# NVlabs/nvbio

Hardware: NVIDIA H100
Metric: Mreads/s (150bp) seed+extend (higher is better)
Workload: dtype int32

## Files before the change

include/nvbio_b200_debug.h:

```cpp
#ifndef NVBIO_B200_DEBUG_H
#define NVBIO_B200_DEBUG_H
#include <stdint.h>
#ifdef __cplusplus
extern "C" {
#endif

void nvb_debug_force_gotoh_path(int path);
int nvb_debug_gotoh_last_route(int* packed, uint32_t* n_int32);
void nvb_debug_full_minb(int minb);
void nvb_debug_full_warp(int mode);
void nvb_debug_full_traceback_warp(int on);
void nvb_debug_pair_format(int on);
void nvb_debug_pair_rows2(int on);
void nvb_debug_traceback_fast(int on);
void nvb_debug_pair_extra_smem(int bytes);

void nvb_debug_pipeline_path(int path);

void nvb_debug_seed_split(int on);
int nvb_debug_seed_todo(uint32_t* n);

void nvb_debug_perfect_shortcut(int on);
int nvb_debug_dp_jobs(uint32_t* n);

int nvb_debug_mapq_eval(const int32_t* d_best, const uint8_t* d_has_second, const int32_t* d_second, const uint32_t* d_len,
                        const int32_t* d_match_bonus, const int32_t* d_min_score, uint32_t n, uint8_t* d_mapq, void* stream);

void nvb_debug_bgzf_grid(uint32_t ctas);

#ifdef __cplusplus
}
#endif
#endif
```

nvbio_b200/_lib.py:

```python
import ctypes as C
import os

_HERE = os.path.dirname(os.path.abspath(__file__))
LIB_PATH = os.environ.get("NVBIO_B200_LIB") or os.path.join(_HERE, "libnvbio_b200.so")

EXPORTS = [
    "nvb_version", "nvb_error_string",
    "nvb_fm_rank", "nvb_fm_rank4", "nvb_fm_match", "nvb_fm_match_approx", "nvb_fm_locate", "nvb_fm_filter_rank", "nvb_fm_filter_locate",
    "nvb_banded_gotoh_score", "nvb_banded_gotoh_score_indirect", "nvb_banded_gotoh_traceback", "nvb_gotoh_score", "nvb_gotoh_score_indirect", "nvb_banded_gotoh_score_window", "nvb_banded_gotoh_score_best2", "nvb_gotoh_traceback", "nvb_seed_extend_paired",
    "nvb_fm_build_occ", "nvb_fm_build_bwt", "nvb_fm_build_ktab", "nvb_fm_build_ktab_located", "nvb_fm_build_ktab_context", "nvb_fm_build_ktab_wide", "nvb_fm_build_rows", "nvb_seed_extend", "nvb_seed_extend_traceback", "nvb_seed_extend_mapq", "nvb_seed_extend_reseed", "nvb_seed_extend_all", "nvb_seed_extend_paired_mapq", "nvb_seed_extend_paired_traceback", "nvb_seed_extend_paired_reseed",
    "nvb_seed_extend_stage_ms",
    "nvb_dict_rank", "nvb_dict_rank4", "nvb_dict_build_occ",
    "nvb_map_seeds", "nvb_fm_locate_init", "nvb_fm_locate_lookup", "nvb_fm_locate_sorted",
    "nvb_pipeline_create", "nvb_pipeline_submit", "nvb_pipeline_wait", "nvb_pipeline_traffic", "nvb_pipeline_destroy",
    "nvb_finish_alignments", "nvb_bam_records", "nvb_bam_records_all", "nvb_bgzf_compress", "nvb_bam_sort", "nvb_bam_index", "nvb_sam_format",
]
DEBUG_EXPORTS = [
    "nvb_debug_gotoh_last_route", "nvb_debug_force_gotoh_path", "nvb_debug_full_minb", "nvb_debug_full_warp", "nvb_debug_full_traceback_warp",
    "nvb_debug_pair_format", "nvb_debug_pair_rows2", "nvb_debug_traceback_fast", "nvb_debug_pair_extra_smem",
    "nvb_debug_pipeline_path", "nvb_debug_seed_split", "nvb_debug_seed_todo", "nvb_debug_perfect_shortcut", "nvb_debug_dp_jobs", "nvb_debug_mapq_eval",
    "nvb_debug_bgzf_grid",
]


class NvbError(RuntimeError):
    pass


class FmIndexStruct(C.Structure):
    _fields_ = [("d_bwt_occ", C.c_void_p), ("d_ssa", C.c_void_p), ("length", C.c_uint32),
                ("primary", C.c_uint32), ("L2", C.c_uint32 * 5), ("sa_interval", C.c_uint32),
                ("d_ktab", C.c_void_p), ("ktab_k", C.c_uint32), ("ktab_located", C.c_uint32), ("d_rows", C.c_void_p)]


class StringSetStruct(C.Structure):
    _fields_ = [("d_words", C.c_void_p), ("bits", C.c_uint32), ("big_endian", C.c_uint32),
                ("d_offsets", C.c_void_p), ("d_lengths", C.c_void_p), ("stride", C.c_uint32),
                ("length", C.c_uint32)]


class GotohSchemeStruct(C.Structure):
    _fields_ = [("match", C.c_int32), ("mismatch", C.c_int32), ("pattern_gap_open", C.c_int32),
                ("pattern_gap_ext", C.c_int32), ("text_gap_open", C.c_int32), ("text_gap_ext", C.c_int32),
                ("d_qual_table", C.c_void_p), ("qual_table_min", C.c_int32), ("qual_table_max", C.c_int32)]


class SeedExtendParamsStruct(C.Structure):
    _fields_ = [("seed_len", C.c_uint32), ("seed_interval", C.c_uint32), ("band_len", C.c_uint32),
                ("type", C.c_uint32), ("both_strands", C.c_uint32), ("max_seed_hits", C.c_uint32),
                ("dedup_jobs", C.c_uint32), ("scheme", GotohSchemeStruct), ("d_read_quals", C.c_void_p)]


class BestAlignmentOutStruct(C.Structure):
    _fields_ = [("d_ops", C.c_void_p), ("max_ops", C.c_uint32), ("d_n_ops", C.c_void_p), ("d_begin", C.c_void_p),
                ("d_strand", C.c_void_p)]


class FinishOutStruct(C.Structure):
    _fields_ = [("d_cigar", C.c_void_p), ("max_cigar", C.c_uint32), ("d_n_cigar", C.c_void_p), ("d_md", C.c_void_p), ("max_md", C.c_uint32),
                ("d_md_len", C.c_void_p), ("d_edits", C.c_void_p)]


class BamInStruct(C.Structure):
    _fields_ = [("reads", StringSetStruct), ("d_read_quals", C.c_void_p), ("d_n_ops", C.c_void_p), ("d_begin", C.c_void_p),
                ("d_strand", C.c_void_p), ("finish", FinishOutStruct), ("d_score", C.c_void_p), ("d_mapq", C.c_void_p),
                ("d_second_score", C.c_void_p), ("d_pair_flags", C.c_void_p), ("d_contig_begin", C.c_void_p), ("n_contigs", C.c_uint32),
                ("d_names", C.c_void_p), ("d_name_offsets", C.c_void_p)]


class BamAllInStruct(C.Structure):
    _fields_ = [("base", BamInStruct), ("d_first", C.c_void_p), ("capacity", C.c_uint32)]


class BamOutStruct(C.Structure):
    _fields_ = [("d_records", C.c_void_p), ("capacity", C.c_uint64), ("d_offsets", C.c_void_p), ("d_counts", C.c_void_p)]


class BgzfOutStruct(C.Structure):
    _fields_ = [("d_out", C.c_void_p), ("capacity", C.c_uint64), ("d_block_offsets", C.c_void_p)]


class BamSortOutStruct(C.Structure):
    _fields_ = [("d_records", C.c_void_p), ("capacity", C.c_uint64), ("d_offsets", C.c_void_p), ("d_order", C.c_void_p)]


class BaiOutStruct(C.Structure):
    _fields_ = [("d_bai", C.c_void_p), ("capacity", C.c_uint64), ("d_size", C.c_void_p), ("d_status", C.c_void_p)]


class SamOutStruct(C.Structure):
    _fields_ = [("d_text", C.c_void_p), ("capacity", C.c_uint64), ("d_offsets", C.c_void_p), ("d_rejected", C.c_void_p)]


class MapqParamsStruct(C.Structure):
    _fields_ = [("d_min_score", C.c_void_p), ("max_read_len", C.c_uint32), ("match_bonus", C.c_int32)]


class MapqOutStruct(C.Structure):
    _fields_ = [("d_second_score", C.c_void_p), ("d_second_pos", C.c_void_p), ("d_second_strand", C.c_void_p), ("d_mapq", C.c_void_p)]


class ReseedParamsStruct(C.Structure):
    _fields_ = [("max_reseed", C.c_uint32), ("rep_seeds", C.c_uint32), ("d_min_score", C.c_void_p), ("max_read_len", C.c_uint32)]


class ReseedOutStruct(C.Structure):
    _fields_ = [("d_rounds", C.c_void_p), ("d_active", C.c_void_p)]


class AllParamsStruct(C.Structure):
    _fields_ = [("max_per_read", C.c_uint32), ("capacity", C.c_uint32)]


class AllOutStruct(C.Structure):
    _fields_ = [("d_first", C.c_void_p), ("d_read", C.c_void_p), ("d_score", C.c_void_p), ("d_pos", C.c_void_p),
                ("alignment", BestAlignmentOutStruct), ("d_count", C.c_void_p)]


class PairParamsStruct(C.Structure):
    _fields_ = [("min_frag", C.c_uint32), ("max_frag", C.c_uint32), ("min_mate_score", C.c_int32), ("rescue_capacity", C.c_uint32)]


class PairOutStruct(C.Structure):
    _fields_ = [("d_pair_score", C.c_void_p), ("d_pair_flags", C.c_void_p), ("d_mate_score", C.c_void_p), ("d_mate_pos", C.c_void_p),
                ("d_mate_strand", C.c_void_p), ("d_n_rescue", C.c_void_p)]


class PairMapqOutStruct(C.Structure):
    _fields_ = [("d_second_pair_score", C.c_void_p), ("d_second_mate_pos", C.c_void_p), ("d_second_mate_strand", C.c_void_p),
                ("d_mate_second_score", C.c_void_p), ("d_mate_mapq", C.c_void_p)]


class PipelineResultStruct(C.Structure):
    _fields_ = [("best_score", C.c_void_p), ("best_pos", C.c_void_p), ("n_hits", C.c_void_p), ("pair_score", C.c_void_p),
                ("pair_flags", C.c_void_p), ("mate_score", C.c_void_p), ("mate_pos", C.c_void_p), ("mate_strand", C.c_void_p),
                ("n_rescue", C.c_void_p), ("device_ms", C.c_float)]


_lib = None


def lib():
    global _lib
    if _lib is None:
        if not os.path.exists(LIB_PATH):
            raise NvbError("nvbio_b200: %s is missing -- run `python -m nvbio_b200.build` "
                           "(there is no CPU fallback)" % LIB_PATH)
        _lib = C.CDLL(LIB_PATH)
        _lib.nvb_error_string.restype = C.c_char_p
        _lib.nvb_pipeline_destroy.restype = None
        _lib.nvb_pipeline_traffic.restype = None
        for name in EXPORTS + DEBUG_EXPORTS:
            getattr(_lib, name)
    return _lib


def check(err, what=""):
    if err != 0:
        msg = lib().nvb_error_string(C.c_int(err)).decode()
        raise NvbError("%s failed: %s (%d)" % (what or "nvbio_b200 call", msg, err))
```

nvbio_b200/csrc/pipeline.cu:

```cuda
#include "fm_core.cuh"
#include "gotoh_core.cuh"
#include "pipeline_core.cuh"
#include "gotoh_full_core.cuh"
#include <cub/agent/single_pass_scan_operators.cuh>
#include <cub/block/block_scan.cuh>
#include <cub/device/device_scan.cuh>
#include <cub/device/device_select.cuh>
#include <cub/device/device_segmented_sort.cuh>
#include <mutex>

namespace nvb {

struct PipeGeom {
    uint32_t n_reads;
    uint32_t n_strings;
    uint32_t strands;
    uint32_t stride;
    uint32_t bits;
    uint32_t seeds_per_string;
    uint32_t seed_len, seed_interval;
    uint32_t band;
    uint32_t max_seed_hits;
    uint32_t genome_len;
    uint32_t seed_offset;
};

template <int BITS>
__global__ void __launch_bounds__(256)
pipe_make_strings_kernel(const StrSet reads, const PipeGeom g, uint32_t* __restrict__ out_words, uint32_t* __restrict__ out_len)
{
    constexpr uint32_t SPW = 32 / BITS;
    const uint32_t words_per_string = g.stride / SPW;
    const uint64_t t = (uint64_t)blockIdx.x * 256 + threadIdx.x;
    if (t >= (uint64_t)g.n_strings * words_per_string) return;
    const uint32_t s = (uint32_t)(t / words_per_string), w = (uint32_t)(t % words_per_string);
    const uint32_t read = s / g.strands, strand = s % g.strands;
    const uint32_t off = str_off(reads, read), len = str_len(reads, read);
    if (w == 0) out_len[s] = len;
    uint32_t word = 0;
    for (uint32_t k = 0; k < SPW; ++k) {
        const uint32_t p = w * SPW + k;
        uint32_t c = 0;
        if (p < len) {
            if (strand == 0) c = sym_at_rt(reads.words, reads.bits, reads.big_endian, off + p);
            else { c = sym_at_rt(reads.words, reads.bits, reads.big_endian, off + (len - 1u - p)); c = (c < 4u) ? 3u - c : c; }
        }
        word |= c << (32u - BITS - BITS * k);
    }
    out_words[t] = word;
}

__global__ void __launch_bounds__(256)
pipe_make_quals_kernel(const StrSet reads, const PipeGeom g, const uint8_t* __restrict__ quals, uint8_t* __restrict__ out)
{
    const uint64_t t = (uint64_t)blockIdx.x * 256 + threadIdx.x;
    if (t >= (uint64_t)g.n_strings * g.stride) return;
    const uint32_t s = (uint32_t)(t / g.stride), p = (uint32_t)(t % g.stride);
    const uint32_t read = s / g.strands, strand = s % g.strands;
    const uint32_t off = str_off(reads, read), len = str_len(reads, read);
    out[t] = (p < len) ? quals[off + (strand == 0 ? p : len - 1u - p)] : (uint8_t)0;
}

__device__ __forceinline__ uint32_t load16_2bit_be(const uint32_t* __restrict__ words, uint32_t p , uint32_t cnt )
{
    const uint32_t w = p >> 4, sh = 2u * (p & 15u);
    const uint32_t a = words[w];
    if (sh == 0) return a;
    const uint32_t b = ((p & 15u) + cnt > 16u) ? words[w + 1] : 0u;
    return (a << sh) | (b >> (32u - sh));
}
__device__ __forceinline__ uint32_t revcomp16_2bit(uint32_t x)
{
    uint32_t y = __brev(~x);
    return ((y >> 1) & 0x55555555u) | ((y & 0x55555555u) << 1);
}
__global__ void __launch_bounds__(256)
pipe_make_strings_2bit_be_kernel(const StrSet reads, const PipeGeom g, uint32_t* __restrict__ out_words, uint32_t* __restrict__ out_len)
{
    const uint32_t words_per_string = g.stride / 16u;
    const uint64_t t = (uint64_t)blockIdx.x * 256 + threadIdx.x, total = (uint64_t)g.n_strings * words_per_string;
    if (t >= total) return;
    uint32_t s, w;
    if (total <= 0xFFFFFFFFull) { s = (uint32_t)t / words_per_string; w = (uint32_t)t - s * words_per_string; }
    else                        { s = (uint32_t)(t / words_per_string); w = (uint32_t)(t % words_per_string); }
    const uint32_t read = s / g.strands, strand = s % g.strands;
    const uint32_t off = str_off(reads, read), len = str_len(reads, read);
    if (w == 0) out_len[s] = len;
    const uint32_t first = w * 16u;
    uint32_t word = 0;
    if (first < len) {
        const uint32_t cnt = (len - first) < 16u ? (len - first) : 16u;
        if (strand == 0) {
            word = load16_2bit_be(reads.words, off + first, cnt);
        } else {
            const uint32_t lo = len - first - cnt;
            uint32_t x = load16_2bit_be(reads.words, off + lo, cnt);
            x = revcomp16_2bit(x);
            word = x << (2u * (16u - cnt));
        }
        if (cnt < 16u) word &= ~(0xFFFFFFFFu >> (2u * cnt));
    }
    out_words[t] = word;
}

__device__ __forceinline__ uint32_t seed_range_hits(uint2 range, uint32_t max_seed_hits)
{
    const uint32_t sz = (range.y == 0xFFFFFFFFu) ? 1u : ((range.x <= range.y) ? (range.y - range.x + 1u) : 0u);
    return sz < max_seed_hits ? sz : max_seed_hits;
}

__device__ __forceinline__ uint2 hit_window(uint32_t pos, uint32_t seed_begin, uint32_t len, const PipeGeom& g)
{
    const uint32_t diag = pos > seed_begin ? pos - seed_begin : 0u;
    const uint32_t gb = diag > g.band / 2u ? diag - g.band / 2u : 0u;
    const uint64_t ge64 = (uint64_t)gb + len + g.band;
    return make_uint2(gb, ge64 < g.genome_len ? (uint32_t)ge64 : g.genome_len);
}

constexpr uint32_t SEED_BLOCK = 128;
constexpr uint32_t SEED_TODO_LISTS = 64;
constexpr uint32_t SEED_TODO_PITCH = 32;
constexpr uint32_t SEED_ITER = 8;
template <int BITS, bool DEFER>
__global__ void __launch_bounds__(SEED_BLOCK, 2048 / SEED_BLOCK)
pipe_seed_match_kernel(const FmIndex f, const PipeGeom g, const uint32_t* __restrict__ words, const uint32_t* __restrict__ slen,
                       const uint32_t* __restrict__ genome, uint2* __restrict__ ranges, uint32_t* __restrict__ sizes,
                       uint32_t* __restrict__ todo, uint32_t* __restrict__ todo_count)
{
    constexpr uint32_t ITER = DEFER ? SEED_ITER : 1u;
#pragma unroll 1
    for (uint32_t it = 0; it < ITER; ++it) {
        const uint32_t q = (blockIdx.x * ITER + it) * SEED_BLOCK + threadIdx.x;
        const bool live = q < g.n_strings * g.seeds_per_string;
        if (!DEFER && !live) return;
        uint32_t x = 1, y = 0;
        bool deferred = false;
        if (live) {
            const uint32_t s = q / g.seeds_per_string, k = q % g.seeds_per_string;
            const uint32_t len = slen[s];
            const uint32_t pos = g.seed_offset + k * g.seed_interval;
            if (pos + g.seed_len <= len) {
                if (genome) {
                    const uint32_t st = fm_match_locate_one<BITS, true, DEFER ? FM_DEFER : FM_WHOLE>(f, genome, words, s * g.stride + pos, g.seed_len, x, y);
                    if (st == FM_EMPTY) { x = 1; y = 0; }
                    deferred = DEFER && st == FM_DEFERRED;
                } else
                    fm_match_one<BITS, true>(f, words, s * g.stride + pos, g.seed_len, 0u, x, y);
            }
            ranges[q] = make_uint2(x, y);
            if (sizes && !deferred) sizes[q] = seed_range_hits(make_uint2(x, y), g.max_seed_hits);
        }
        if (DEFER) {
            const uint32_t m = __ballot_sync(0xFFFFFFFFu, deferred);
            if (m) {
                const uint32_t lane = threadIdx.x & 31u, list = blockIdx.x % SEED_TODO_LISTS;
                const uint32_t cap = ((gridDim.x + SEED_TODO_LISTS - 1u) / SEED_TODO_LISTS) * SEED_BLOCK * SEED_ITER;
                uint32_t base = 0;
                if (lane == 0) base = atomicAdd(todo_count + list * SEED_TODO_PITCH, (uint32_t)__popc(m));
                base = __shfl_sync(0xFFFFFFFFu, base, 0);
                if (deferred) todo[(size_t)list * cap + base + __popc(m & ((1u << lane) - 1u))] = q;
            }
        }
    }
}
template <int BITS>
__global__ void __launch_bounds__(SEED_BLOCK, 2048 / SEED_BLOCK)
pipe_seed_match_wide_kernel(const FmIndex f, const PipeGeom g, const uint32_t* __restrict__ words,
                            const uint32_t* __restrict__ genome, uint2* __restrict__ ranges, uint32_t* __restrict__ sizes,
                            const uint32_t* __restrict__ todo, const uint32_t* __restrict__ todo_count, const uint32_t seed_grid)
{
    const uint32_t list = blockIdx.x % SEED_TODO_LISTS, per_list = gridDim.x / SEED_TODO_LISTS;
    const uint32_t cap = ((seed_grid + SEED_TODO_LISTS - 1u) / SEED_TODO_LISTS) * SEED_BLOCK * SEED_ITER;
    const uint32_t n = todo_count[list * SEED_TODO_PITCH];
    for (uint32_t t = (blockIdx.x / SEED_TODO_LISTS) * SEED_BLOCK + threadIdx.x; t < n; t += per_list * SEED_BLOCK) {
        const uint32_t q = todo[(size_t)list * cap + t];
        const uint32_t s = q / g.seeds_per_string, k = q % g.seeds_per_string;
        const uint2 r = ranges[q];
        uint32_t x = r.x, y = r.y;
        if (fm_match_locate_one<BITS, true, FM_RESUME>(f, genome, words, s * g.stride + g.seed_offset + k * g.seed_interval, g.seed_len, x, y) == FM_EMPTY) { x = 1; y = 0; }
        ranges[q] = make_uint2(x, y);
        if (sizes) sizes[q] = seed_range_hits(make_uint2(x, y), g.max_seed_hits);
    }
}

__device__ __forceinline__ uint32_t upper_bound_u32(const uint32_t* __restrict__ a, uint32_t n, uint32_t v)
{
    uint32_t lo = 0, hi = n;
    while (lo < hi) { const uint32_t mid = (lo + hi) >> 1; if (a[mid] <= v) lo = mid + 1; else hi = mid; }
    return lo;
}

__global__ void pipe_count_kernel(const uint32_t* __restrict__ excl, const uint32_t* __restrict__ sizes, uint32_t n_queries, uint32_t capacity,
                                  uint32_t* __restrict__ counts)
{
    if (threadIdx.x == 0 && blockIdx.x == 0) {
        const uint32_t total = n_queries ? excl[n_queries - 1] + sizes[n_queries - 1] : 0u;
        counts[1] = total;
        counts[0] = total < capacity ? total : capacity;
    }
}

__global__ void __launch_bounds__(256)
pipe_expand_hits_kernel(const FmIndex f, const PipeGeom g, const uint2* __restrict__ ranges, const uint32_t* __restrict__ sizes,
                        const uint32_t* __restrict__ excl, const uint32_t* __restrict__ slen, const uint32_t* __restrict__ counts,
                        uint32_t* __restrict__ hit_string, uint32_t* __restrict__ p_off, uint32_t* __restrict__ p_len,
                        uint32_t* __restrict__ t_off, uint32_t* __restrict__ t_len)
{
    const uint32_t q = blockIdx.x * 256 + threadIdx.x;
    if (q >= g.n_strings * g.seeds_per_string) return;
    const uint32_t sz = sizes[q];
    if (sz == 0) return;
    const uint32_t base = excl[q], kept = counts[0];
    const uint32_t x = ranges[q].x;
    const uint32_t s = q / g.seeds_per_string, k = q % g.seeds_per_string;
    const uint32_t seed_begin = g.seed_offset + k * g.seed_interval;
    const uint32_t len = slen[s];
    for (uint32_t j = 0; j < sz; ++j) {
        const uint32_t h = base + j;
        if (h >= kept) break;
        const uint2 w = hit_window(fm_locate_one(f, x + j), seed_begin, len, g);
        hit_string[h] = s;
        p_off[h] = s * g.stride; p_len[h] = len;
        t_off[h] = w.x;          t_len[h] = w.y - w.x;
    }
}

struct Jobs { uint32_t *p_off, *p_len, *t_off, *t_len; };

constexpr uint32_t RJ_BLOCK = 128;
constexpr uint32_t RJ_STAGE = 640;
constexpr int      RJ_LOCAL = 6;
constexpr uint32_t RJ_BATCH = 4;
constexpr uint32_t RJ_CLAIMED = 0xFFFFFFFFu, RJ_CLAIMED_EMPTY = 0xFFFFFFFEu;
using RjTileState = cub::ScanTileState<uint32_t>;
using RjPrefixOp  = cub::TilePrefixCallbackOp<uint32_t, ::cuda::std::plus<uint32_t>, RjTileState>;

template <uint32_t RB>
__device__ __forceinline__ uint32_t range_batch(const uint2* __restrict__ rr, const uint32_t q0, const uint32_t n, const bool vec,
                                                const uint32_t max_seed_hits, uint32_t& hits)
{
    uint2 v[RB];
    if (vec) {
#pragma unroll
        for (uint32_t j = 0; j < RB; j += 2u) {
            const uint4 w = q0 + j < n ? *reinterpret_cast<const uint4*>(rr + q0 + j) : make_uint4(1u, 0u, 1u, 0u);
            v[j] = make_uint2(w.x, w.y); v[j + 1] = make_uint2(w.z, w.w);
        }
    } else {
#pragma unroll
        for (uint32_t j = 0; j < RB; ++j) v[j] = q0 + j < n ? rr[q0 + j] : make_uint2(1u, 0u);
    }
    uint32_t m = 0;
#pragma unroll
    for (uint32_t j = 0; j < RB; ++j) {
        const uint32_t sz = seed_range_hits(v[j], max_seed_hits);
        hits += sz;
        m |= (sz != 0u ? 1u : 0u) << j;
    }
    return m;
}

__global__ void __launch_bounds__(256)
pipe_resolve_init_kernel(RjTileState tiles, const uint32_t n_tiles, uint32_t* __restrict__ counts, uint32_t* __restrict__ dp_count)
{
    tiles.InitializeStatus((int)n_tiles);
    if (blockIdx.x == 0 && threadIdx.x == 0) { counts[2] = 0u; counts[3] = 0u; *dp_count = 0u; }
}

__global__ void __launch_bounds__(RJ_BLOCK, 8)
pipe_resolve_reads_kernel(const FmIndex f, const PipeGeom g, const uint2* __restrict__ ranges, const uint32_t* __restrict__ slen,
                          const uint32_t hit_capacity, RjTileState tiles, const uint32_t n_tiles, uint32_t* __restrict__ counts,
                          const int shortcut, const int32_t match, const int32_t mismatch, const int32_t max_gap_open,
                          const uint32_t* __restrict__ str_words, const uint32_t* __restrict__ genome,
                          uint32_t* __restrict__ j_string, uint32_t* __restrict__ j_first, const Jobs jobs,
                          int32_t* __restrict__ job_score, uint2* __restrict__ job_sink,
                          const Jobs dp, uint32_t* __restrict__ dp_job, uint32_t* __restrict__ dp_count,
                          unsigned long long* __restrict__ best_key, int32_t* best_score, uint32_t* best_pos, uint8_t* __restrict__ best_strand)
{
    using BlockScan = cub::BlockScan<uint32_t, RJ_BLOCK>;
    __shared__ struct { typename RjPrefixOp::TempStorage prefix; typename BlockScan::TempStorage scan; } s_tmp;
    __shared__ uint32_t st_string[RJ_STAGE], st_first[RJ_STAGE], st_toff[RJ_STAGE], st_tlen[RJ_STAGE], st_slot[RJ_STAGE];
    __shared__ unsigned long long s_key[RJ_BLOCK];
    __shared__ int32_t s_score[RJ_BLOCK];
    __shared__ uint32_t s_pos[RJ_BLOCK];
    __shared__ uint8_t s_strand[RJ_BLOCK];
    __shared__ uint32_t s_tile, s_cnt, s_base, s_dp_cnt, s_dp_base;
    if (threadIdx.x == 0) { s_tile = atomicAdd(counts + 3, 1u); s_cnt = 0u; s_dp_cnt = 0u; }
    s_key[threadIdx.x] = 0ull;
    __syncthreads();
    const uint32_t tile = s_tile, r0 = tile * RJ_BLOCK, r = r0 + threadIdx.x;
    const uint32_t per_read = g.strands * g.seeds_per_string;
    const bool live = r < g.n_reads;
    const uint2* rr = ranges + (size_t)r * per_read;

    const bool vec = ((per_read | (uint32_t)((size_t)ranges >> 3)) & 1u) == 0u;
    uint32_t hits = 0, run = 0, nonempty = 0;
    if (live)
        for (uint32_t q0 = 0; q0 < per_read; q0 += 16u) {
            const uint32_t m = range_batch<16>(rr, q0, per_read, vec, g.max_seed_hits, hits);
            if (q0 < 32u) nonempty |= m << q0;
        }
    if (tile == 0) {
        uint32_t aggregate;
        BlockScan(s_tmp.scan).ExclusiveSum(hits, run, aggregate);
        if (threadIdx.x == 0) tiles.SetInclusive(0, aggregate);
    } else {
        RjPrefixOp prefix(tiles, s_tmp.prefix, ::cuda::std::plus<uint32_t>{}, (int)tile);
        BlockScan(s_tmp.scan).ExclusiveSum(hits, run, prefix);
    }
    if (tile == n_tiles - 1u && threadIdx.x == RJ_BLOCK - 1u) {
        const uint32_t total = run + hits;
        counts[1] = total;
        counts[0] = total < hit_capacity ? total : hit_capacity;
    }

    if (live) {
        uint32_t lk_s[RJ_LOCAL], lk_b[RJ_LOCAL], lk_e[RJ_LOCAL];
        int n_local = 0;
        const uint32_t len0 = slen[r * g.strands], len1 = g.strands > 1u ? slen[r * g.strands + 1u] : 0u;
        for (uint32_t q0 = 0; q0 < per_read; q0 += 32u) {
            uint32_t m = q0 ? 0u : nonempty, unused = 0;
            if (q0)
                for (uint32_t b = 0; b < 32u; b += 8u) m |= range_batch<8>(rr, q0 + b, per_read, vec, g.max_seed_hits, unused) << b;
            while (m) {
                uint32_t bq[RJ_BATCH], nb = 0;
                uint2 brq[RJ_BATCH];
#pragma unroll
                for (uint32_t e = 0; e < RJ_BATCH; ++e) { bq[e] = m ? q0 + (uint32_t)__ffs(m) - 1u : 0u; nb += m ? 1u : 0u; m &= m - 1u; }
#pragma unroll
                for (uint32_t e = 0; e < RJ_BATCH; ++e) brq[e] = e < nb ? rr[bq[e]] : make_uint2(1u, 0u);
                for (uint32_t e = 0; e < nb; ++e) {
                    const uint32_t q = bq[0];
                    const uint2 rq = brq[0];
#pragma unroll
                    for (uint32_t c = 0; c + 1u < RJ_BATCH; ++c) { bq[c] = bq[c + 1]; brq[c] = brq[c + 1]; }
                    const uint32_t strand = q < g.seeds_per_string ? 0u : 1u, k = q - strand * g.seeds_per_string;
                    const uint32_t s = r * g.strands + strand, len = strand ? len1 : len0;
                    const bool located = rq.y == 0xFFFFFFFFu;
                    const uint32_t sz = seed_range_hits(rq, g.max_seed_hits);
                    const uint32_t base = run, x = rq.x, seed_begin = g.seed_offset + k * g.seed_interval;
                    run += sz;
                    for (uint32_t j = 0; j < sz; ++j) {
                        const uint32_t h = base + j;
                        if (h >= hit_capacity) break;
                        const uint2 w = hit_window(located ? x : fm_locate_one(f, x + j), seed_begin, len, g);
                        bool seen = false;
#pragma unroll
                        for (int e = 0; e < RJ_LOCAL; ++e) seen |= (e < n_local) && lk_s[e] == s && lk_b[e] == w.x && lk_e[e] == w.y;
                        if (seen) continue;
#pragma unroll
                        for (int e = 0; e < RJ_LOCAL; ++e) if (e == n_local) { lk_s[e] = s; lk_b[e] = w.x; lk_e[e] = w.y; }
                        if (n_local < RJ_LOCAL) ++n_local;
                        const uint32_t slot = atomicAdd(&s_cnt, 1u);
                        if (slot < RJ_STAGE) { st_string[slot] = s; st_first[slot] = h; st_toff[slot] = w.x; st_tlen[slot] = w.y - w.x; }
                        else {
                            const uint32_t o = atomicAdd(counts + 2, 1u), d = atomicAdd(dp_count, 1u);
                            j_string[o] = s; j_first[o] = h;
                            jobs.p_off[o] = s * g.stride; jobs.p_len[o] = len; jobs.t_off[o] = w.x; jobs.t_len[o] = w.y - w.x;
                            dp.p_off[d] = s * g.stride; dp.p_len[d] = len; dp.t_off[d] = w.x; dp.t_len[d] = w.y - w.x; dp_job[d] = o;
                        }
                    }
                }
            }
        }
    }
    __syncthreads();

    const uint32_t n = s_cnt < RJ_STAGE ? s_cnt : RJ_STAGE;
    if (threadIdx.x == 0) s_base = n ? atomicAdd(counts + 2, n) : 0u;
    __syncthreads();
    for (uint32_t i = threadIdx.x; i < n; i += RJ_BLOCK) {
        const uint32_t o = s_base + i, s = st_string[i], first = st_first[i], len = slen[s], to = st_toff[i], N = st_tlen[i];
        j_string[o] = s; j_first[o] = first; jobs.p_off[o] = s * g.stride; jobs.p_len[o] = len; jobs.t_off[o] = to; jobs.t_len[o] = N;
        int32_t score = 0; uint32_t sx = 0, sy = 0;
        if (shortcut && gapless_job_shortcut(str_words, genome, s * g.stride, len, to, N, g.band, match, mismatch, max_gap_open, score, sx, sy,
                                             shortcut != 2)) {
            const uint2 sk = make_uint2(sx, sy);
            job_score[o] = score; job_sink[o] = sk;
            if (job_aligned(sk)) {
                st_slot[i] = RJ_CLAIMED; st_toff[i] = to + sx; st_tlen[i] = (uint32_t)score;
                atomicMax(&s_key[s / g.strands - r0], make_best_key(score, first));
            } else st_slot[i] = RJ_CLAIMED_EMPTY;
        } else st_slot[i] = atomicAdd(&s_dp_cnt, 1u);
    }
    __syncthreads();
    if (threadIdx.x == 0) s_dp_base = s_dp_cnt ? atomicAdd(dp_count, s_dp_cnt) : 0u;
    __syncthreads();
    for (uint32_t i = threadIdx.x; i < n; i += RJ_BLOCK) {
        const uint32_t slot = st_slot[i], s = st_string[i];
        if (slot == RJ_CLAIMED) {
            const uint32_t rl = s / g.strands - r0;
            const int32_t score = (int32_t)st_tlen[i];
            if (s_key[rl] == make_best_key(score, st_first[i])) { s_score[rl] = score; s_pos[rl] = st_toff[i]; s_strand[rl] = (uint8_t)(s % g.strands); }
        } else if (slot != RJ_CLAIMED_EMPTY) {
            const uint32_t d = s_dp_base + slot;
            dp.p_off[d] = s * g.stride; dp.p_len[d] = slen[s]; dp.t_off[d] = st_toff[i]; dp.t_len[d] = st_tlen[i]; dp_job[d] = s_base + i;
        }
    }
    __syncthreads();
    if (live) {
        const unsigned long long key = s_key[threadIdx.x];
        best_key[r] = key;
        best_score[r] = key ? s_score[threadIdx.x] : INT_MIN;
        best_pos[r] = key ? s_pos[threadIdx.x] : 0xFFFFFFFFu;
        best_strand[r] = key ? s_strand[threadIdx.x] : (uint8_t)0;
    }
}

__global__ void __launch_bounds__(256)
pipe_scatter_dp_kernel(const PipeGeom g, const uint32_t* __restrict__ dp_count, const uint32_t* __restrict__ dp_job,
                       const int32_t* __restrict__ dp_score, const uint2* __restrict__ dp_sink,
                       const uint32_t* __restrict__ j_string, const uint32_t* __restrict__ j_first,
                       int32_t* __restrict__ job_score, uint2* __restrict__ job_sink, unsigned long long* __restrict__ best_key)
{
    const uint32_t n = *dp_count;
    for (uint32_t a = blockIdx.x * 256 + threadIdx.x; a < n; a += gridDim.x * 256) {
        const uint32_t j = dp_job[a];
        const int32_t sc = dp_score[a];
        const uint2 sk = dp_sink[a];
        job_score[j] = sc; job_sink[j] = sk;
        if (job_aligned(sk)) atomicMax(best_key + j_string[j] / g.strands, make_best_key(sc, j_first[j]));
    }
}

__global__ void __launch_bounds__(256)
pipe_finalize_dp_kernel(const PipeGeom g, const uint32_t* __restrict__ dp_count, const uint32_t* __restrict__ dp_job,
                        const int32_t* __restrict__ dp_score, const uint2* __restrict__ dp_sink, const uint32_t* __restrict__ dp_t_off,
                        const uint32_t* __restrict__ j_string, const uint32_t* __restrict__ j_first,
                        const unsigned long long* __restrict__ best_key,
                        int32_t* __restrict__ best_score, uint32_t* __restrict__ best_pos, uint8_t* __restrict__ best_strand)
{
    const uint32_t n = *dp_count;
    for (uint32_t a = blockIdx.x * 256 + threadIdx.x; a < n; a += gridDim.x * 256) {
        const uint32_t j = dp_job[a], s = j_string[j], read = s / g.strands;
        const int32_t sc = dp_score[a];
        if (best_key[read] != make_best_key(sc, j_first[j])) continue;
        best_score[read] = sc; best_pos[read] = dp_t_off[a] + dp_sink[a].x; best_strand[read] = (uint8_t)(s % g.strands);
    }
}

__global__ void __launch_bounds__(256)
pipe_find_leaders_kernel(const uint32_t* __restrict__ counts, const uint32_t* __restrict__ hit_string,
                         const uint32_t* __restrict__ t_off, const uint32_t* __restrict__ t_len,
                         uint32_t* __restrict__ leader, uint32_t* __restrict__ flag)
{
    constexpr uint32_t BACK = 64u;
    __shared__ uint32_t ss[256 + BACK], so[256 + BACK], sl[256 + BACK];
    const uint32_t n = counts[0];
    const uint32_t h0 = blockIdx.x * 256;
    if (h0 >= n) return;
    for (uint32_t i = threadIdx.x; i < 256 + BACK; i += 256) {
        const int64_t g = (int64_t)h0 - BACK + i;
        const bool in = g >= 0 && g < (int64_t)n;
        ss[i] = in ? hit_string[g] : 0xFFFFFFFFu; so[i] = in ? t_off[g] : 0u; sl[i] = in ? t_len[g] : 0u;
    }
    __syncthreads();
    const uint32_t h = h0 + threadIdx.x;
    if (h >= n) return;
    const uint32_t me = threadIdx.x + BACK;
    const uint32_t s = ss[me], o = so[me], l = sl[me];
    uint32_t lead = h;
    for (uint32_t back = 1; back <= BACK && back <= h; ++back) {
        if (ss[me - back] != s) break;
        if (so[me - back] == o && sl[me - back] == l) lead = h - back;
    }
    leader[h] = lead;
    flag[h] = (lead == h) ? 1u : 0u;
}

__global__ void pipe_job_count_kernel(const uint32_t* __restrict__ job_idx, const uint32_t* __restrict__ flag, uint32_t* __restrict__ counts)
{
    if (threadIdx.x == 0 && blockIdx.x == 0) {
        const uint32_t n = counts[0];
        counts[2] = n ? job_idx[n - 1] + flag[n - 1] : 0u;
    }
}

__global__ void __launch_bounds__(256)
pipe_compact_jobs_kernel(const uint32_t* __restrict__ counts, const uint32_t* __restrict__ flag, const uint32_t* __restrict__ job_idx,
                         const uint32_t* __restrict__ p_off, const uint32_t* __restrict__ p_len,
                         const uint32_t* __restrict__ t_off, const uint32_t* __restrict__ t_len,
                         uint32_t* __restrict__ jp_off, uint32_t* __restrict__ jp_len, uint32_t* __restrict__ jt_off, uint32_t* __restrict__ jt_len)
{
    const uint32_t h = blockIdx.x * 256 + threadIdx.x;
    if (h >= counts[0] || !flag[h]) return;
    const uint32_t j = job_idx[h];
    jp_off[j] = p_off[h]; jp_len[j] = p_len[h]; jt_off[j] = t_off[h]; jt_len[j] = t_len[h];
}

__global__ void __launch_bounds__(256)
pipe_scatter_scores_kernel(const PipeGeom g, const uint32_t* __restrict__ counts, const uint32_t* __restrict__ leader, const uint32_t* __restrict__ job_idx,
                           const int32_t* __restrict__ job_score, const uint2* __restrict__ job_sink, const uint32_t* __restrict__ hit_string,
                           int32_t* __restrict__ score, uint2* __restrict__ sink, unsigned long long* __restrict__ best_key)
{
    const uint32_t h = blockIdx.x * 256 + threadIdx.x;
    if (h >= counts[0]) return;
    uint32_t l = leader[h];
    for (uint32_t nx = leader[l]; nx != l; nx = leader[l]) l = nx;
    const uint32_t j = job_idx[l];
    const int32_t sc = job_score[j];
    const uint2 sk = job_sink[j];
    score[h] = sc;
    sink[h]  = sk;
    if (job_aligned(sk)) atomicMax(best_key + hit_string[h] / g.strands, make_best_key(sc, h));
}

__global__ void __launch_bounds__(256)
pipe_reduce_kernel(const PipeGeom g, const uint32_t* __restrict__ counts, const uint32_t* __restrict__ hit_string,
                   const int32_t* __restrict__ score, const uint2* __restrict__ sink, unsigned long long* __restrict__ best_key)
{
    const uint32_t h = blockIdx.x * 256 + threadIdx.x;
    if (h >= counts[0] || !job_aligned(sink[h])) return;
    atomicMax(best_key + hit_string[h] / g.strands, make_best_key(score[h], h));
}

__global__ void __launch_bounds__(256)
pipe_finalize_kernel(const PipeGeom g, const unsigned long long* __restrict__ best_key, const uint32_t* __restrict__ t_off,
                     const uint2* __restrict__ sink, const uint32_t* __restrict__ hit_string,
                     int32_t* __restrict__ best_score, uint32_t* __restrict__ best_pos, uint8_t* __restrict__ best_strand)
{
    const uint32_t r = blockIdx.x * 256 + threadIdx.x;
    if (r >= g.n_reads) return;
    const unsigned long long key = best_key[r];
    if (key == 0ull) { best_score[r] = INT_MIN; best_pos[r] = 0xFFFFFFFFu; if (best_strand) best_strand[r] = 0; return; }
    const uint32_t h = best_key_index(key);
    best_score[r] = best_key_score(key);
    best_pos[r] = t_off[h] + sink[h].x;
    if (best_strand) best_strand[r] = (uint8_t)(hit_string[h] % g.strands);
}

__global__ void __launch_bounds__(256)
pipe_best_jobs_kernel(const PipeGeom g, const unsigned long long* __restrict__ best_key, const uint32_t* __restrict__ hit_string,
                      const uint32_t* __restrict__ p_off, const uint32_t* __restrict__ p_len,
                      const uint32_t* __restrict__ t_off, const uint32_t* __restrict__ t_len,
                      uint32_t* __restrict__ bp_off, uint32_t* __restrict__ bp_len, uint32_t* __restrict__ bt_off, uint32_t* __restrict__ bt_len,
                      uint8_t* __restrict__ strand)
{
    const uint32_t r = blockIdx.x * 256 + threadIdx.x;
    if (r >= g.n_reads) return;
    const unsigned long long key = best_key[r];
    if (key == 0ull) { bp_off[r] = 0; bp_len[r] = 0; bt_off[r] = 0; bt_len[r] = 0; if (strand) strand[r] = 0; return; }
    const uint32_t h = best_key_index(key);
    bp_off[r] = p_off[h]; bp_len[r] = p_len[h]; bt_off[r] = t_off[h]; bt_len[r] = t_len[h];
    if (strand) strand[r] = (uint8_t)(hit_string[h] % g.strands);
}

struct Scored {
    const uint32_t* count; const uint32_t* string; const uint32_t* tie_index; Jobs jobs; const int32_t* score; const uint2* sink;
    __device__ __forceinline__ uint32_t tie(uint32_t j) const { return tie_index ? tie_index[j] : j; }
    __device__ __forceinline__ uint32_t end(uint32_t j) const { return jobs.t_off[j] + sink[j].x; }
};

__global__ void __launch_bounds__(256)
pipe_empty_jobs_kernel(const uint32_t n_reads, uint32_t* __restrict__ bp_off, uint32_t* __restrict__ bp_len, uint32_t* __restrict__ bt_off,
                       uint32_t* __restrict__ bt_len, uint8_t* __restrict__ strand)
{
    const uint32_t r = blockIdx.x * 256 + threadIdx.x;
    if (r >= n_reads) return;
    bp_off[r] = 0; bp_len[r] = 0; bt_off[r] = 0; bt_len[r] = 0;
    if (strand) strand[r] = 0;
}

__global__ void __launch_bounds__(256)
pipe_winner_kernel(const PipeGeom g, const Scored c, const unsigned long long* __restrict__ key, const Jobs out,
                   uint32_t* __restrict__ end, uint8_t* __restrict__ strand)
{
    const uint32_t n = *c.count;
    for (uint32_t j = blockIdx.x * 256 + threadIdx.x; j < n; j += gridDim.x * 256) {
        const uint32_t s = c.string[j], r = s / g.strands;
        if (key[r] != make_best_key(c.score[j], c.tie(j))) continue;
        if (out.p_off) { out.p_off[r] = c.jobs.p_off[j]; out.p_len[r] = c.jobs.p_len[j]; out.t_off[r] = c.jobs.t_off[j]; out.t_len[r] = c.jobs.t_len[j]; }
        if (end) end[r] = c.end(j);
        if (strand) strand[r] = (uint8_t)(s % g.strands);
    }
}

__global__ void __launch_bounds__(256)
traceback_begin_kernel(const uint32_t* __restrict__ d_n, const uint32_t n, const unsigned long long* __restrict__ best_key,
                       const uint32_t* __restrict__ t_off, const uint2* __restrict__ source, uint32_t* __restrict__ n_ops, uint2* __restrict__ begin)
{
    const uint32_t i = blockIdx.x * 256 + threadIdx.x;
    if (i >= (d_n ? *d_n : n)) return;
    if (best_key && best_key[i] == 0ull) { n_ops[i] = 0; begin[i] = make_uint2(0xFFFFFFFFu, 0xFFFFFFFFu); return; }
    const uint2 sc = source[i];
    begin[i] = make_uint2(t_off[i] + sc.x, sc.y);
}

__global__ void __launch_bounds__(256)
pipe_export_hits_kernel(const PipeGeom g, const uint32_t* __restrict__ counts, const uint32_t* __restrict__ hit_string,
                        const uint32_t* __restrict__ t_off, const uint32_t* __restrict__ t_len,
                        uint32_t* __restrict__ out_read, uint2* __restrict__ out_window)
{
    const uint32_t h = blockIdx.x * 256 + threadIdx.x;
    if (h >= counts[0]) return;
    if (out_read)   out_read[h] = hit_string[h];
    if (out_window) out_window[h] = make_uint2(t_off[h], t_off[h] + t_len[h]);
}


__global__ void __launch_bounds__(256)
reseed_fold_kernel(const PipeGeom g, const Scored c, const uint32_t* __restrict__ map, const uint32_t base, const uint32_t t0,
                   uint32_t* __restrict__ u_string, uint32_t* __restrict__ u_tie, const Jobs u, int32_t* __restrict__ u_score,
                   uint2* __restrict__ u_sink, unsigned long long* __restrict__ key)
{
    const uint32_t n = *c.count;
    for (uint32_t j = blockIdx.x * 256 + threadIdx.x; j < n; j += gridDim.x * 256) {
        const uint32_t s = c.string[j], read = map ? map[s / g.strands] : s / g.strands, os = read * g.strands + s % g.strands;
        const uint32_t o = base + j, tie = t0 + c.tie(j);
        const int32_t sc = c.score[j];
        const uint2 sk = c.sink[j];
        u_string[o] = os; u_tie[o] = tie;
        u.p_off[o] = os * g.stride; u.p_len[o] = c.jobs.p_len[j]; u.t_off[o] = c.jobs.t_off[j]; u.t_len[o] = c.jobs.t_len[j];
        u_score[o] = sc; u_sink[o] = sk;
        if (job_aligned(sk)) atomicMax(key + read, make_best_key(sc, tie));
    }
}

__global__ void __launch_bounds__(256)
reseed_flag_kernel(const PipeGeom g, const uint2* __restrict__ ranges, const uint32_t* __restrict__ map, const uint32_t* __restrict__ str_len,
                   const unsigned long long* __restrict__ key, const int32_t* __restrict__ min_score, const uint32_t rep_seeds,
                   uint8_t* __restrict__ flag)
{
    const uint32_t i = blockIdx.x * 256 + threadIdx.x;
    if (i >= g.n_reads) return;
    const uint32_t per_read = g.strands * g.seeds_per_string;
    const uint2* rr = ranges + (size_t)i * per_read;
    uint32_t range_sum = 0u, range_count = 0u;
    for (uint32_t q = 0; q < per_read; ++q) {
        const uint2 v = rr[q];
        if (v.y != 0xFFFFFFFFu && v.x > v.y) continue;
        range_sum += v.y == 0xFFFFFFFFu ? 1u : v.y - v.x + 1u;
        ++range_count;
    }
    bool aligned = true;
    if (min_score) {
        const unsigned long long k = key[map ? map[i] : i];
        aligned = k != 0ull && best_key_score(k) >= min_score[str_len[i * g.strands]];
    }
    flag[i] = reseed_read(range_sum, range_count, rep_seeds, aligned) ? 1u : 0u;
}

__global__ void __launch_bounds__(256)
reseed_gather_kernel(const PipeGeom g, const uint32_t* __restrict__ map, const uint32_t* __restrict__ words0, const uint32_t* __restrict__ len0,
                     const uint8_t* __restrict__ quals0, uint32_t* __restrict__ words, uint32_t* __restrict__ len, uint8_t* __restrict__ quals,
                     uint8_t* __restrict__ rounds, const uint32_t round)
{
    const uint32_t spw = 32u / g.bits, wps = g.stride / spw;
    const uint64_t t = (uint64_t)blockIdx.x * 256 + threadIdx.x;
    if (t >= (uint64_t)g.n_strings * wps) return;
    const uint32_t s = (uint32_t)(t / wps), w = (uint32_t)(t % wps), read = map[s / g.strands], os = read * g.strands + s % g.strands;
    words[t] = words0[(size_t)os * wps + w];
    if (quals)
        for (uint32_t b = 0; b < spw; ++b) quals[(size_t)s * g.stride + w * spw + b] = quals0[(size_t)os * g.stride + w * spw + b];
    if (w == 0) {
        len[s] = len0[os];
        if (rounds && s % g.strands == 0u) rounds[read] = (uint8_t)(round + 1u);
    }
}

__global__ void __launch_bounds__(256)
reseed_export_hits_kernel(const PipeGeom g, const uint32_t* __restrict__ counts, const uint32_t* __restrict__ map,
                          const uint32_t* __restrict__ hit_string, const uint32_t* __restrict__ t_off, const uint32_t* __restrict__ t_len,
                          uint32_t* __restrict__ out_read, uint2* __restrict__ out_window)
{
    const uint32_t h = blockIdx.x * 256 + threadIdx.x;
    if (h >= counts[0]) return;
    const uint32_t s = hit_string[h];
    if (out_read)   out_read[h] = (map ? map[s / g.strands] : s / g.strands) * g.strands + s % g.strands;
    if (out_window) out_window[h] = make_uint2(t_off[h], t_off[h] + t_len[h]);
}

__global__ void reseed_counts_kernel(const uint32_t* __restrict__ counts, const bool dedup, const bool per_read, uint32_t* __restrict__ totals,
                                     uint32_t* __restrict__ active, const uint32_t round, const uint32_t n_round)
{
    if (threadIdx.x != 0 || blockIdx.x != 0) return;
    const uint32_t jobs = dedup ? (counts[0] ? counts[2] : 0u) : counts[0];
    totals[0] += counts[0]; totals[1] += counts[1]; totals[2] += jobs; totals[3] += per_read ? jobs : counts[0];
    if (active) active[round] = n_round;
}

__global__ void __launch_bounds__(256)
reseed_best_kernel(const uint32_t n_reads, const unsigned long long* __restrict__ key, int32_t* __restrict__ best_score,
                   uint32_t* __restrict__ best_pos, uint8_t* __restrict__ best_strand)
{
    const uint32_t r = blockIdx.x * 256 + threadIdx.x;
    if (r >= n_reads) return;
    const unsigned long long k = key[r];
    best_score[r] = k ? best_key_score(k) : INT_MIN;
    best_pos[r] = 0xFFFFFFFFu; best_strand[r] = 0;
}

__global__ void __launch_bounds__(256) reseed_iota_kernel(const uint32_t n, uint32_t* __restrict__ map)
{
    const uint32_t i = blockIdx.x * 256 + threadIdx.x;
    if (i < n) map[i] = i;
}


__device__ __forceinline__ bool second_candidate(int32_t score, uint32_t end, uint32_t strand, uint32_t len, uint32_t best_end,
                                                 uint32_t best_strand, const int32_t* __restrict__ min_score)
{
    return score >= min_score[len] && distinct_alignment(end, strand, best_end, best_strand, len);
}

__global__ void __launch_bounds__(256)
pipe_second_reduce_kernel(const PipeGeom g, const Scored c, const uint32_t* __restrict__ str_len, const uint32_t* __restrict__ best_pos,
                          const uint8_t* __restrict__ best_strand, const int32_t* __restrict__ min_score,
                          unsigned long long* __restrict__ second_key)
{
    const uint32_t n = *c.count;
    for (uint32_t j = blockIdx.x * 256 + threadIdx.x; j < n; j += gridDim.x * 256) {
        const uint32_t s = c.string[j], read = s / g.strands;
        const int32_t sc = c.score[j];
        if (job_aligned(c.sink[j]) && second_candidate(sc, c.end(j), s % g.strands, str_len[s], best_pos[read], best_strand[read], min_score))
            atomicMax(second_key + read, make_best_key(sc, c.tie(j)));
    }
}

__global__ void __launch_bounds__(256)
pipe_mapq_kernel(const PipeGeom g, const nvb_mapq_params mp, const uint32_t* __restrict__ str_len, const int32_t* __restrict__ best_score,
                 const unsigned long long* __restrict__ second_key, int32_t* __restrict__ second_score, uint32_t* __restrict__ second_pos,
                 uint8_t* __restrict__ second_strand, uint8_t* __restrict__ mapq)
{
    const uint32_t r = blockIdx.x * 256 + threadIdx.x;
    if (r >= g.n_reads) return;
    const unsigned long long key = second_key[r];
    const bool has = key != 0ull;
    const int32_t s2 = has ? best_key_score(key) : INT_MIN;
    second_score[r] = s2;
    if (!has) {
        if (second_pos) second_pos[r] = 0xFFFFFFFFu;
        if (second_strand) second_strand[r] = 0;
    }
    const uint32_t len = str_len[r * g.strands];
    mapq[r] = (uint8_t)bowtie_mapq2(best_score[r], has, s2, (int32_t)len * mp.match_bonus, mp.d_min_score[len], mp.match_bonus == 0);
}

__global__ void __launch_bounds__(256)
debug_mapq_eval_kernel(const int32_t* __restrict__ best, const uint8_t* __restrict__ has_second, const int32_t* __restrict__ second,
                       const uint32_t* __restrict__ len, const int32_t* __restrict__ match_bonus, const int32_t* __restrict__ min_score,
                       uint32_t n, uint8_t* __restrict__ mapq)
{
    const uint32_t i = blockIdx.x * 256 + threadIdx.x;
    if (i >= n) return;
    mapq[i] = (uint8_t)bowtie_mapq2(best[i], has_second[i] != 0, second[i], (int32_t)len[i] * match_bonus[i], min_score[i], match_bonus[i] == 0);
}

__global__ void __launch_bounds__(256)
cand_scatter_kernel(const PipeGeom g, const Scored c, const uint32_t* __restrict__ str_len, const int32_t* __restrict__ min_score,
                    const uint32_t* __restrict__ seg, uint32_t* __restrict__ cursor, unsigned long long* __restrict__ key,
                    uint32_t* __restrict__ val, const bool by_best)
{
    const uint32_t n = *c.count;
    for (uint32_t j = blockIdx.x * 256 + threadIdx.x; j < n; j += gridDim.x * 256) {
        const uint32_t s = c.string[j], read = s / g.strands;
        if (!reportable(c.score[j], c.sink[j], min_score[str_len[s]])) continue;
        const uint32_t slot = atomicAdd(cursor + read, 1u);
        if (!seg) continue;
        key[seg[read] + slot] = by_best ? ~make_best_key(c.score[j], c.tie(j)) : ((unsigned long long)(s % g.strands) << 32) | c.end(j);
        val[seg[read] + slot] = j;
    }
}


__global__ void __launch_bounds__(256)
all_select_kernel(const PipeGeom g, const Scored c, const uint32_t* __restrict__ str_len, const uint32_t* __restrict__ seg,
                  unsigned long long* __restrict__ es, uint32_t* __restrict__ idx, const uint32_t k, uint32_t* __restrict__ cnt)
{
    const uint32_t r = blockIdx.x * 256 + threadIdx.x;
    if (r >= g.n_reads) return;
    const uint32_t b = seg[r], n = seg[r + 1] - b;
    for (uint32_t i = 0; i < n; ++i) {
        const uint32_t j = idx[b + i];
        es[b + i] = end_strand(c.end(j), c.string[j] % g.strands);
    }
    cnt[r] = select_distinct(es + b, idx + b, n, str_len[r * g.strands], k);
}

__global__ void __launch_bounds__(256)
all_count_kernel(const uint32_t n_reads, const uint32_t* __restrict__ first, const uint32_t capacity, const uint32_t n_slices,
                 uint32_t* __restrict__ count, uint32_t* __restrict__ slice_n)
{
    const uint32_t stored = first[upper_bound_u32(first, n_reads + 1u, capacity) - 1u];
    const uint32_t t = blockIdx.x * 256 + threadIdx.x;
    if (t == 0) { count[0] = stored; count[1] = first[n_reads]; }
    if (t >= n_slices) return;
    const uint64_t b = (uint64_t)t * n_reads;
    slice_n[t] = stored > b ? (uint32_t)(stored - b < n_reads ? stored - b : n_reads) : 0u;
}

__global__ void __launch_bounds__(256)
all_emit_kernel(const PipeGeom g, const Scored c, const uint32_t* __restrict__ first, const uint32_t* __restrict__ seg,
                const uint32_t* __restrict__ idx, const uint32_t capacity, uint32_t* __restrict__ out_read, int32_t* __restrict__ out_score,
                uint32_t* __restrict__ out_pos, uint8_t* __restrict__ out_strand, const Jobs jobs)
{
    const uint32_t r = blockIdx.x * 256 + threadIdx.x;
    if (r >= g.n_reads) return;
    const uint32_t o = first[r], e = first[r + 1];
    if (e > capacity) return;
    const uint32_t* sel = idx + seg[r];
    for (uint32_t a = o; a < e; ++a) {
        const uint32_t j = sel[a - o], s = c.string[j];
        out_read[a] = r; out_score[a] = c.score[j]; out_pos[a] = c.end(j); out_strand[a] = (uint8_t)(s % g.strands);
        jobs.p_off[a] = c.jobs.p_off[j]; jobs.p_len[a] = c.jobs.p_len[j]; jobs.t_off[a] = c.jobs.t_off[j]; jobs.t_len[a] = c.jobs.t_len[j];
    }
}

struct MateBest { bool has; int32_t score; uint32_t strand, beg, end, len; };

__device__ __forceinline__ MateBest mate_best(const PipeGeom& g, uint32_t r, const int32_t* best_score,
                                              const uint32_t* best_pos, const uint8_t* __restrict__ best_strand,
                                              const uint32_t* __restrict__ str_len)
{
    MateBest m; m.has = false; m.score = INT_MIN; m.strand = 0; m.beg = m.end = 0xFFFFFFFFu; m.len = 0;
    const uint32_t end = best_pos[r];
    if (end == 0xFFFFFFFFu) return m;
    m.has = true;
    m.score = best_score[r];
    m.strand = best_strand[r];
    m.len = str_len[r * g.strands];
    m.end = end;
    m.beg = aln_begin(m.end, m.len);
    return m;
}

__global__ void __launch_bounds__(256)
pair_classify_kernel(const PipeGeom g, const uint32_t n_pairs, const nvb_pair_params pp,
                     const int32_t* best_score, const uint32_t* best_pos, const uint8_t* __restrict__ best_strand,
                     const uint32_t* __restrict__ str_len,
                     uint32_t* __restrict__ want, uint32_t* __restrict__ w_pstr, uint32_t* __restrict__ w_toff, uint32_t* __restrict__ w_tlen,
                     int32_t* __restrict__ pair_score, uint32_t* __restrict__ pair_flags,
                     int32_t* mate_score, uint32_t* mate_pos, uint8_t* __restrict__ mate_strand)
{
    const uint32_t p = blockIdx.x * 256 + threadIdx.x;
    if (p >= n_pairs) return;
    MateBest m[2];
    m[0] = mate_best(g, p, best_score, best_pos, best_strand, str_len);
    m[1] = mate_best(g, n_pairs + p, best_score, best_pos, best_strand, str_len);
#pragma unroll
    for (int k = 0; k < 2; ++k) {
        mate_score[k * n_pairs + p] = m[k].score; mate_pos[k * n_pairs + p] = m[k].end; mate_strand[k * n_pairs + p] = (uint8_t)m[k].strand;
    }
    bool conc = m[0].has && m[1].has && (m[0].strand != m[1].strand);
    if (conc) {
        const MateBest& f = m[0].strand == 0 ? m[0] : m[1];
        const MateBest& r = m[0].strand == 0 ? m[1] : m[0];
        conc = fr_concordant(f.beg, f.end, r.beg, r.end, pp.min_frag, pp.max_frag);
    }
    if (conc) {
        pair_score[p] = m[0].score + m[1].score; pair_flags[p] = NVB_PAIR_CONCORDANT;
        want[2 * p] = want[2 * p + 1] = 0u;
        return;
    }
    pair_score[p] = INT_MIN; pair_flags[p] = NVB_PAIR_UNPAIRED;
#pragma unroll
    for (int a = 0; a < 2; ++a) {
        uint32_t w = 0u, ps = 0u, to = 0u, tl = 0u;
        if (m[a].has && m[a].score >= pp.min_mate_score) {
            const uint32_t o_read = (uint32_t)(1 - a) * n_pairs + p;
            if (m[a].strand == 0u) { to = m[a].beg; const uint32_t e = (g.genome_len - to) < pp.max_frag ? g.genome_len : to + pp.max_frag; tl = e - to; ps = 2u * o_read + 1u; }
            else                   { to = m[a].end > pp.max_frag ? m[a].end - pp.max_frag : 0u; tl = m[a].end - to; ps = 2u * o_read; }
            w = (tl >= 1u && str_len[ps] >= 1u) ? 1u : 0u;
        }
        want[2 * p + a] = w; w_pstr[2 * p + a] = ps; w_toff[2 * p + a] = to; w_tlen[2 * p + a] = tl;
    }
}

__global__ void __launch_bounds__(256)
pair_compact_kernel(const PipeGeom g, const uint32_t n_slots, const uint32_t capacity, const uint32_t* __restrict__ want, const uint32_t* __restrict__ job_idx,
                    const uint32_t* __restrict__ w_pstr, const uint32_t* __restrict__ w_toff, const uint32_t* __restrict__ w_tlen,
                    const uint32_t* __restrict__ str_len,
                    uint32_t* __restrict__ jp_off, uint32_t* __restrict__ jp_len, uint32_t* __restrict__ jt_off, uint32_t* __restrict__ jt_len)
{
    const uint32_t i = blockIdx.x * 256 + threadIdx.x;
    if (i >= n_slots || !want[i]) return;
    const uint32_t j = job_idx[i];
    if (j >= capacity) return;
    jp_off[j] = w_pstr[i] * g.stride; jp_len[j] = str_len[w_pstr[i]]; jt_off[j] = w_toff[i]; jt_len[j] = w_tlen[i];
}

__device__ __forceinline__ bool usable_rescue(const nvb_pair_params& pp, const uint32_t* __restrict__ want, const uint32_t* __restrict__ job_idx,
                                              const uint32_t* __restrict__ w_toff, const int32_t* __restrict__ rs_score,
                                              const uint2* __restrict__ rs_sink, uint32_t i, int32_t& score, uint32_t& end)
{
    if (!want[i]) return false;
    const uint32_t j = job_idx[i];
    if (j >= pp.rescue_capacity) return false;
    score = rs_score[j];
    if (score < pp.min_mate_score) return false;
    end = w_toff[i] + rs_sink[j].x;
    return true;
}

__global__ void __launch_bounds__(256)
pair_finalize_kernel(const uint32_t n_pairs, const nvb_pair_params pp, const uint32_t* __restrict__ want, const uint32_t* __restrict__ job_idx,
                     const uint32_t* __restrict__ w_toff, const int32_t* __restrict__ rs_score, const uint2* __restrict__ rs_sink,
                     int32_t* __restrict__ pair_score, uint32_t* __restrict__ pair_flags,
                     int32_t* __restrict__ mate_score, uint32_t* __restrict__ mate_pos, uint8_t* __restrict__ mate_strand)
{
    const uint32_t p = blockIdx.x * 256 + threadIdx.x;
    if (p >= n_pairs || pair_flags[p] == NVB_PAIR_CONCORDANT) return;
    int best_a = -1; int32_t best_sum = INT_MIN, best_rs = 0; uint32_t best_pos = 0;
#pragma unroll
    for (int a = 0; a < 2; ++a) {
        int32_t rs; uint32_t end;
        if (!usable_rescue(pp, want, job_idx, w_toff, rs_score, rs_sink, 2 * p + a, rs, end)) continue;
        const int32_t sum = mate_score[a * n_pairs + p] + rs;
        if (sum > best_sum) { best_sum = sum; best_a = a; best_rs = rs; best_pos = end; }
    }
    if (best_a < 0) return;
    const int o = 1 - best_a;
    pair_score[p] = best_sum;
    pair_flags[p] = o == 0 ? NVB_PAIR_RESCUED_MATE1 : NVB_PAIR_RESCUED_MATE2;
    mate_score[o * n_pairs + p] = best_rs;
    mate_pos[o * n_pairs + p] = best_pos;
    mate_strand[o * n_pairs + p] = (uint8_t)(1u - mate_strand[best_a * n_pairs + p]);
}

__device__ __forceinline__ bool pair_rescued(uint32_t flags) { return flags == NVB_PAIR_RESCUED_MATE1 || flags == NVB_PAIR_RESCUED_MATE2; }

__global__ void __launch_bounds__(256)
pair_empty_rescued_jobs_kernel(const uint32_t n_pairs, const uint32_t* __restrict__ pair_flags, uint32_t* __restrict__ bp_len, uint32_t* __restrict__ bt_len)
{
    const uint32_t p = blockIdx.x * 256 + threadIdx.x;
    if (p >= n_pairs) return;
    const uint32_t f = pair_flags[p];
    if (!pair_rescued(f)) return;
    const uint32_t r = (f == NVB_PAIR_RESCUED_MATE1 ? 0u : n_pairs) + p;
    bp_len[r] = 0; bt_len[r] = 0;
}

__global__ void __launch_bounds__(256)
pair_rescue_items_kernel(const uint32_t n_pairs, const uint32_t* __restrict__ pair_flags, const uint32_t* __restrict__ job_idx,
                         const uint8_t* __restrict__ mate_strand, uint2* __restrict__ items, uint32_t* __restrict__ n_items, uint8_t* __restrict__ ba_strand)
{
    const uint32_t p = blockIdx.x * 256 + threadIdx.x, lane = threadIdx.x & 31u;
    const uint32_t f = p < n_pairs ? pair_flags[p] : 0u;
    const bool rescued = pair_rescued(f);
    const uint32_t m = __ballot_sync(0xFFFFFFFFu, rescued);
    if (!m) return;
    uint32_t base = 0;
    if (lane == 0) base = atomicAdd(n_items, (uint32_t)__popc(m));
    base = __shfl_sync(0xFFFFFFFFu, base, 0);
    if (!rescued) return;
    const uint32_t o = f == NVB_PAIR_RESCUED_MATE1 ? 0u : 1u, out = o * n_pairs + p;
    items[base + __popc(m & ((1u << lane) - 1u))] = make_uint2(job_idx[2u * p + (1u - o)], out);
    if (ba_strand) ba_strand[out] = mate_strand[out];
}


__global__ void __launch_bounds__(256)
pair_cand_merge_kernel(const uint32_t n_reads, const uint32_t* __restrict__ seg, const uint32_t* __restrict__ cnt,
                       const unsigned long long* __restrict__ key, const uint32_t* __restrict__ val, const Scored c,
                       uint32_t* __restrict__ m_end, int32_t* __restrict__ m_score, uint32_t* __restrict__ m_tie,
                       uint32_t* __restrict__ n_fw, uint32_t* __restrict__ n_merged)
{
    const uint32_t r = blockIdx.x * 256 + threadIdx.x;
    if (r >= n_reads) return;
    const uint32_t b = seg[r], n = cnt[r];
    uint32_t m = 0, fw = 0; unsigned long long prev = ~0ull;
    for (uint32_t k = b; k < b + n; ++k) {
        const unsigned long long kk = key[k];
        const uint32_t j = val[k], tie = c.tie(j);
        const int32_t sc = c.score[j];
        if (kk == prev) {
            const uint32_t o = b + m - 1u;
            if (sc > m_score[o] || (sc == m_score[o] && tie < m_tie[o])) { m_score[o] = sc; m_tie[o] = tie; }
            continue;
        }
        prev = kk;
        m_end[b + m] = (uint32_t)kk; m_score[b + m] = sc; m_tie[b + m] = tie;
        ++m; if ((kk >> 32) == 0ull) ++fw;
    }
    n_fw[r] = fw; n_merged[r] = m;
}

__global__ void __launch_bounds__(256)
pair_second_kernel(const uint32_t n_pairs, const nvb_pair_params pp, const nvb_mapq_params mp, const uint32_t* __restrict__ str_len,
                   const uint32_t* __restrict__ seg, const uint32_t* __restrict__ n_fw, const uint32_t* __restrict__ n_merged,
                   const uint32_t* __restrict__ m_end, const int32_t* __restrict__ m_score, const uint32_t* __restrict__ m_tie,
                   const uint32_t* __restrict__ se_pos, const uint8_t* __restrict__ se_strand, const unsigned long long* __restrict__ best_key,
                   const uint32_t* __restrict__ want, const uint32_t* __restrict__ job_idx, const uint32_t* __restrict__ w_toff,
                   const int32_t* __restrict__ rs_score, const uint2* __restrict__ rs_sink,
                   const int32_t* __restrict__ pair_score, const uint32_t* __restrict__ pair_flags,
                   const uint32_t* __restrict__ mate_pos, const uint8_t* __restrict__ mate_strand,
                   int32_t* __restrict__ second_pair_score, uint32_t* __restrict__ second_mate_pos, uint8_t* __restrict__ second_mate_strand,
                   uint8_t* __restrict__ mate_mapq)
{
    const uint32_t p = blockIdx.x * 256 + threadIdx.x;
    if (p >= n_pairs) return;
    const uint32_t r0 = p, r1 = n_pairs + p;
    const uint32_t len[2] = {str_len[2u * r0], str_len[2u * r1]};
    PairSecond ps;
    ps.init(mate_pos[r0], mate_strand[r0], len[0], mate_pos[r1], mate_strand[r1], len[1]);
    const uint32_t flags = pair_flags[p];
    if (flags != NVB_PAIR_UNPAIRED) {
        MateCands m[2];
#pragma unroll
        for (int k = 0; k < 2; ++k) {
            const uint32_t r = k ? r1 : r0, b = seg[r];
            m[k].end = m_end + b; m[k].score = m_score + b; m[k].tie = m_tie + b; m[k].n_fw = n_fw[r]; m[k].n = n_merged[r]; m[k].len = len[k];
        }
        pair_combinations(m, pp.min_frag, pp.max_frag, ps);
        for (int a = 0; a < 2; ++a) {
            const uint32_t ra = a ? r1 : r0;
            int32_t rs; uint32_t end;
            if (!usable_rescue(pp, want, job_idx, w_toff, rs_score, rs_sink, 2u * p + a, rs, end) || rs < mp.d_min_score[len[1 - a]]) continue;
            const unsigned long long key = best_key[ra];
            ps.offer_rescue(a, best_key_score(key) + rs, se_pos[ra], se_strand[ra], best_key_index(key), end);
        }
        const uint8_t q = (uint8_t)bowtie_mapq2(pair_score[p], ps.has, ps.score, (int32_t)(len[0] + len[1]) * mp.match_bonus,
                                                mp.d_min_score[len[0]] + mp.d_min_score[len[1]], mp.match_bonus == 0);
        mate_mapq[r0] = q; mate_mapq[r1] = q;
    }
    second_pair_score[p] = ps.score;
#pragma unroll
    for (int k = 0; k < 2; ++k) {
        if (second_mate_pos) second_mate_pos[k * n_pairs + p] = ps.end[k];
        if (second_mate_strand) second_mate_strand[k * n_pairs + p] = (uint8_t)ps.strand[k];
    }
}

}

using namespace nvb;

struct StageEvents { cudaEvent_t ev[8]; bool ready, valid; };
static StageEvents g_stage[NVB_MAX_DEVICES];
static std::mutex  g_stage_mutex;
static int default_stage_events(StageEvents** out)
{
    int dev = 0;
    NVB_CUDA_TRY(cudaGetDevice(&dev));
    if (dev < 0 || dev >= NVB_MAX_DEVICES) return NVB_E_UNSUPPORTED;
    std::lock_guard<std::mutex> lock(g_stage_mutex);
    StageEvents& S = g_stage[dev];
    if (!S.ready) {
        for (int i = 0; i < 8; ++i) NVB_CUDA_TRY(cudaEventCreate(&S.ev[i]));
        S.ready = true;
    }
    *out = &S;
    return NVB_OK;
}

extern "C" int nvb_seed_extend_stage_ms(float ms[7])
{
    if (!ms) return NVB_E_INVALID;
    StageEvents* SE = nullptr;
    { const int r = default_stage_events(&SE); if (r != NVB_OK) return r; }
    if (!SE->valid) return NVB_E_INVALID;
    NVB_CUDA_TRY(cudaEventSynchronize(SE->ev[7]));
    for (int i = 0; i < 7; ++i) NVB_CUDA_TRY(cudaEventElapsedTime(&ms[i], SE->ev[i], SE->ev[i + 1]));
    return NVB_OK;
}

static int g_perfect_shortcut = 1;
static const uint32_t* g_last_dp_count = nullptr;
static int g_seed_split = 1;
static const uint32_t* g_last_seed_todo = nullptr;
static int g_pipe_path = 0;

#define NVB_TRY(expr) do { const int _r = (expr); if (_r != NVB_OK) return _r; } while (0)
static int size_only(int r) { return r == NVB_E_TEMP_SIZE ? NVB_OK : r; }
static int launched() { return (int)cudaGetLastError(); }

static uint32_t resident_grid(uint32_t n) { const uint32_t grid = (n + 255) / 256, cap = sm_count() * 16u; return grid < cap ? grid : cap; }

static Jobs take_jobs(TempCarver& tc, size_t n) { return Jobs{tc.take<uint32_t>(n), tc.take<uint32_t>(n), tc.take<uint32_t>(n), tc.take<uint32_t>(n)}; }
struct JobViews { nvb_string_set pats, txts; };

struct SeedExtendReq {
    const nvb_fm_index* fmi; const uint32_t* genome; const nvb_string_set* reads; uint32_t n_reads; const nvb_seed_extend_params* P; uint32_t hit_capacity;
    int32_t* best_score; uint32_t* best_pos; uint32_t* n_hits; uint32_t* hit_read; nvb_uint2* hit_window; int32_t* hit_score; nvb_uint2* hit_sink;
    const nvb_best_alignment_out* BA; const nvb_pair_params* PP; const nvb_pair_out* PO;
    const nvb_mapq_params* MP; const nvb_mapq_out* MO; const nvb_pair_mapq_out* PMO;
    const nvb_all_params* AP; const nvb_all_out* AO;
};

struct PipeCall : SeedExtendReq {
    PipeGeom g; cudaStream_t s; FmIndex f; StrSet rd;
    uint32_t nq;
    bool dedup, per_read, eligible;
    bool seed_split;
    nvb_mapq_out se_mo;
    StageEvents* SE;
    uint32_t *str_words, *str_len; uint8_t* str_quals;
    uint2* ranges; uint32_t *sizes, *excl, *counts, *seed_todo, *seed_todo_n;
    char* rj_tiles; size_t rj_tile_bytes;
    uint32_t *j_string, *j_first;
    uint32_t *leader, *flag, *job_idx;
    Jobs jobs; int32_t* job_score; uint2* job_sink;
    Jobs dp; uint32_t *dp_job, *dp_count; int32_t* dp_score; uint2* dp_sink;
    uint32_t* hit_string; Jobs hits; int32_t* h_score; uint2* h_sink;
    unsigned long long* best_key; uint8_t* rb_strand;
    char *scan_tmp, *gotoh_tmp; size_t scan_bytes, gotoh_bytes;
    Jobs best; int32_t* b_score; uint2 *b_sink, *b_source; char* tb_tmp; size_t tb_bytes;
    uint32_t *pw_want, *pw_idx, *pw_pstr, *pw_toff, *pw_tlen, *pcounts;
    Jobs rescue; int32_t* rs_score; uint2* rs_sink; char *pscan_tmp, *full_tmp; size_t pscan_bytes, full_bytes;
    uint2* rt_items; uint32_t* rt_count; char* rt_pool; size_t rt_pool_bytes;
    unsigned long long* second_key;
    uint32_t *cs_cnt, *cs_seg, *cs_val[2]; unsigned long long* cs_key[2];
    char *cs_scan_tmp, *cs_sort_tmp; size_t cs_scan_bytes, cs_sort_bytes;
    uint32_t *pc_fw, *pc_n, *pc_end, *pc_tie, *se_pos; int32_t* pc_score;
    uint32_t *al_slice_n, n_slices; Jobs al_jobs;
    const Scored* uni;

    int stage(int i) const { return (int)cudaEventRecord(SE->ev[i], s); }

    JobViews job_views(const Jobs& j, uint32_t txt_len) const
    {
        return {{str_words ? str_words : (const uint32_t*)16,  g.bits, 1u,         j.p_off,   j.p_len,   0u,     rd.length},
                {genome,                                       2u,     1u,         j.t_off,   j.t_len,   0u,     txt_len}};
    }

    int score_jobs(const Jobs& j, const uint32_t* d_n, int32_t* score, uint2* sink) const
    {
        const JobViews v = job_views(j, rd.length + g.band);
        size_t bytes = gotoh_bytes;
        return nvb_banded_gotoh_score_indirect(g.band, P->type, &P->scheme, &v.pats, str_quals, &v.txts, d_n, hit_capacity,
                                               score, (nvb_uint2*)sink, gotoh_tmp, &bytes, s);
    }

    int carve(void* d_temp, size_t& need)
    {
        const uint32_t cap = hit_capacity, n_reads = g.n_reads;
        const JobViews sv = job_views(Jobs{}, rd.length + g.band);
        NVB_TRY(size_only(nvb_banded_gotoh_score(g.band, P->type, &P->scheme, &sv.pats, nullptr, &sv.txts, cap, nullptr, nullptr, nullptr,
                                                 &gotoh_bytes, s)));
        TempCarver tc(d_temp);
        str_words = tc.take<uint32_t>((size_t)g.n_strings * (g.stride / (32u / g.bits)) + 4);
        str_len   = tc.take<uint32_t>(g.n_strings);
        str_quals = P->d_read_quals ? tc.take<uint8_t>((size_t)g.n_strings * g.stride + 16) : nullptr;
        ranges = tc.take<uint2>(nq);
        if (!per_read) { sizes = tc.take<uint32_t>(nq); excl = tc.take<uint32_t>(nq); }
        if (seed_split) seed_todo = tc.take<uint32_t>((size_t)nq + (SEED_TODO_LISTS + 1u) * SEED_BLOCK * SEED_ITER);
        counts = tc.take<uint32_t>(4); seed_todo_n = tc.take<uint32_t>(SEED_TODO_LISTS * SEED_TODO_PITCH);
        if (per_read) {
            NVB_CUDA_TRY(RjTileState::AllocationSize((int)((n_reads + RJ_BLOCK - 1u) / RJ_BLOCK), rj_tile_bytes));
            rj_tiles = tc.take<char>(rj_tile_bytes);
        }
        if (per_read) { j_string = tc.take<uint32_t>(cap); j_first = tc.take<uint32_t>(cap); }
        else if (dedup) { leader = tc.take<uint32_t>(cap); flag = tc.take<uint32_t>(cap); job_idx = tc.take<uint32_t>(cap); }
        if (dedup) { jobs = take_jobs(tc, cap); job_score = tc.take<int32_t>(cap); job_sink = tc.take<uint2>(cap); }
        if (per_read) {
            dp = take_jobs(tc, cap); dp_job = tc.take<uint32_t>(cap); dp_score = tc.take<int32_t>(cap); dp_sink = tc.take<uint2>(cap);
            dp_count = tc.take<uint32_t>(4);
        }
        if (!per_read) { hit_string = tc.take<uint32_t>(cap); hits = take_jobs(tc, cap); }
        h_score = hit_score ? hit_score : (per_read ? nullptr : tc.take<int32_t>(cap));
        h_sink  = hit_sink ? (uint2*)hit_sink : (per_read ? nullptr : tc.take<uint2>(cap));
        best_key = tc.take<unsigned long long>(n_reads); rb_strand = tc.take<uint8_t>((size_t)n_reads + 16);
        scan_bytes = 0;
        if (!per_read) NVB_CUDA_TRY(cub::DeviceScan::ExclusiveSum(nullptr, scan_bytes, sizes, excl, (int)nq, s));
        if (dedup && !per_read && cap) {
            size_t scan2_bytes = 0;
            NVB_CUDA_TRY(cub::DeviceScan::ExclusiveSum(nullptr, scan2_bytes, flag, job_idx, (int)cap, s));
            if (scan2_bytes > scan_bytes) scan_bytes = scan2_bytes;
        }
        scan_tmp  = tc.take<char>(scan_bytes);
        gotoh_tmp = tc.take<char>(gotoh_bytes);
        if (BA || AO) {
            if (BA) best = take_jobs(tc, n_reads);
            b_score = tc.take<int32_t>(n_reads); b_sink = tc.take<uint2>(n_reads); b_source = tc.take<uint2>(n_reads);
            NVB_TRY(size_only(nvb_banded_gotoh_traceback(g.band, P->type, &P->scheme, &sv.pats, nullptr, &sv.txts, n_reads, nullptr, nullptr,
                                                         nullptr, nullptr, BA ? BA->max_ops : AO->alignment.max_ops, nullptr, nullptr, &tb_bytes, s)));
            tb_tmp = tc.take<char>(tb_bytes);
        }
        if (PP) {
            const uint32_t rcap = PP->rescue_capacity;
            pw_want = tc.take<uint32_t>(n_reads); pw_idx = tc.take<uint32_t>(n_reads); pw_pstr = tc.take<uint32_t>(n_reads);
            pw_toff = tc.take<uint32_t>(n_reads); pw_tlen = tc.take<uint32_t>(n_reads); pcounts = tc.take<uint32_t>(4);
            rescue = take_jobs(tc, rcap); rs_score = tc.take<int32_t>(rcap); rs_sink = tc.take<uint2>(rcap);
            NVB_CUDA_TRY(cub::DeviceScan::ExclusiveSum(nullptr, pscan_bytes, pw_want, pw_idx, (int)n_reads, s));
            pscan_tmp = tc.take<char>(pscan_bytes);
            const JobViews v = job_views(Jobs{}, PP->max_frag);
            NVB_TRY(size_only(nvb_gotoh_score_indirect(P->type, &P->scheme, &v.pats, nullptr, &v.txts, (const uint32_t*)16, rcap, nullptr, nullptr,
                                                       nullptr, &full_bytes, s)));
            full_tmp = tc.take<char>(full_bytes);
            if (BA) {
                NVB_TRY(full_warp_traceback(P->type, rd.length, PP->max_frag, nullptr, &rt_pool_bytes, s));
                rt_items = tc.take<uint2>((size_t)n_reads / 2u + 1u); rt_count = tc.take<uint32_t>(4); rt_pool = tc.take<char>(rt_pool_bytes);
            }
        }
        if (MO) second_key = tc.take<unsigned long long>(n_reads);
        if (PMO || AO) {
            cs_cnt = tc.take<uint32_t>((size_t)n_reads + 1); cs_seg = tc.take<uint32_t>((size_t)n_reads + 1);
            for (int k = 0; k < 2; ++k) { cs_key[k] = tc.take<unsigned long long>(cap); cs_val[k] = tc.take<uint32_t>(cap); }
            NVB_CUDA_TRY(cub::DeviceScan::ExclusiveSum(nullptr, cs_scan_bytes, cs_cnt, cs_seg, (int)n_reads + 1, s));
            cs_scan_tmp = tc.take<char>(cs_scan_bytes);
            cs_sort_bytes = 0;
            if (cap) NVB_CUDA_TRY(cub::DeviceSegmentedSort::SortPairs(nullptr, cs_sort_bytes, cs_key[0], cs_key[1], cs_val[0], cs_val[1], (int)cap,
                                                                     (int)n_reads, cs_seg, cs_seg + 1, s));
            cs_sort_tmp = tc.take<char>(cs_sort_bytes);
        }
        if (PMO) {
            if (!PMO->d_mate_second_score) se_mo.d_second_score = tc.take<int32_t>(n_reads);
            pc_fw = tc.take<uint32_t>(n_reads); pc_n = tc.take<uint32_t>(n_reads); se_pos = tc.take<uint32_t>(n_reads);
            pc_end = tc.take<uint32_t>(cap); pc_score = tc.take<int32_t>(cap); pc_tie = tc.take<uint32_t>(cap);
        }
        if (AO) {
            const uint32_t acap = AP->capacity;
            n_slices = n_reads ? (uint32_t)(((uint64_t)acap + n_reads - 1u) / n_reads) : 0u;
            al_jobs = take_jobs(tc, acap); al_slice_n = tc.take<uint32_t>((size_t)n_slices + 1);
        }
        need = tc.total();
        return NVB_OK;
    }

    int make_strings() const
    {
        const uint32_t grid = (uint32_t)(((uint64_t)g.n_strings * (g.stride / (32u / g.bits)) + 255) / 256);
        if (g.bits == 2 && rd.big_endian) pipe_make_strings_2bit_be_kernel<<<grid, 256, 0, s>>>(rd, g, str_words, str_len);
        else if (g.bits == 2)             pipe_make_strings_kernel<2><<<grid, 256, 0, s>>>(rd, g, str_words, str_len);
        else                              pipe_make_strings_kernel<4><<<grid, 256, 0, s>>>(rd, g, str_words, str_len);
        NVB_LAUNCH_CHECK();
        if (str_quals) pipe_make_quals_kernel<<<(uint32_t)(((uint64_t)g.n_strings * g.stride + 255) / 256), 256, 0, s>>>(rd, g, P->d_read_quals, str_quals);
        return launched();
    }

    int match_seeds() const
    {
        const uint32_t grid = (nq + SEED_BLOCK - 1) / SEED_BLOCK;
        const uint32_t* loc_genome = (per_read && f.sa_shift == 0u) ? genome : nullptr;
        if (seed_split) {
            NVB_CUDA_TRY(cudaMemsetAsync(seed_todo_n, 0, SEED_TODO_LISTS * SEED_TODO_PITCH * sizeof(uint32_t), s));
            const uint32_t grid1 = (grid + SEED_ITER - 1u) / SEED_ITER;
            if (g.bits == 2) pipe_seed_match_kernel<2, true><<<grid1, SEED_BLOCK, 0, s>>>(f, g, str_words, str_len, loc_genome, ranges, sizes, seed_todo, seed_todo_n);
            else             pipe_seed_match_kernel<4, true><<<grid1, SEED_BLOCK, 0, s>>>(f, g, str_words, str_len, loc_genome, ranges, sizes, seed_todo, seed_todo_n);
            NVB_LAUNCH_CHECK();
            const uint32_t wgrid = (sm_count() * 16u + SEED_TODO_LISTS - 1u) / SEED_TODO_LISTS * SEED_TODO_LISTS;
            if (g.bits == 2) pipe_seed_match_wide_kernel<2><<<wgrid, SEED_BLOCK, 0, s>>>(f, g, str_words, loc_genome, ranges, sizes, seed_todo, seed_todo_n, grid1);
            else             pipe_seed_match_wide_kernel<4><<<wgrid, SEED_BLOCK, 0, s>>>(f, g, str_words, loc_genome, ranges, sizes, seed_todo, seed_todo_n, grid1);
            g_last_seed_todo = seed_todo_n;
        } else {
            if (g.bits == 2) pipe_seed_match_kernel<2, false><<<grid, SEED_BLOCK, 0, s>>>(f, g, str_words, str_len, loc_genome, ranges, sizes, nullptr, nullptr);
            else             pipe_seed_match_kernel<4, false><<<grid, SEED_BLOCK, 0, s>>>(f, g, str_words, str_len, loc_genome, ranges, sizes, nullptr, nullptr);
        }
        return launched();
    }

    int hit_slots() const
    {
        if (per_read) return NVB_OK;
        size_t bytes = scan_bytes;
        NVB_CUDA_TRY(cub::DeviceScan::ExclusiveSum(scan_tmp, bytes, sizes, excl, (int)nq, s));
        pipe_count_kernel<<<1, 32, 0, s>>>(excl, sizes, nq, hit_capacity, counts);
        return launched();
    }

    int extend_per_read() const
    {
        const nvb_gotoh_scheme& SC = P->scheme;
        const uint32_t cap = hit_capacity, n_tiles = (g.n_reads + RJ_BLOCK - 1u) / RJ_BLOCK;
        RjTileState tiles;
        NVB_CUDA_TRY(tiles.Init((int)n_tiles, rj_tiles, rj_tile_bytes));
        pipe_resolve_init_kernel<<<(n_tiles + 255u) / 256u, 256, 0, s>>>(tiles, n_tiles, counts, dp_count);
        NVB_LAUNCH_CHECK();
        const int shortcut = eligible ? g_perfect_shortcut : 0;
        const int32_t max_gap_open = SC.pattern_gap_open > SC.text_gap_open ? SC.pattern_gap_open : SC.text_gap_open;
        pipe_resolve_reads_kernel<<<n_tiles, RJ_BLOCK, 0, s>>>(f, g, ranges, str_len, cap, tiles, n_tiles, counts, shortcut, SC.match,
                SC.mismatch, max_gap_open, str_words, genome, j_string, j_first, jobs, job_score, job_sink, dp, dp_job, dp_count,
                best_key, best_score, best_pos, rb_strand);
        NVB_LAUNCH_CHECK();
        g_last_dp_count = dp_count;
        NVB_TRY(stage(4)); NVB_TRY(stage(5));
        const uint32_t jgrid = resident_grid(cap);
        if (cap) {
            NVB_TRY(score_jobs(dp, dp_count, dp_score, dp_sink));
            pipe_scatter_dp_kernel<<<jgrid, 256, 0, s>>>(g, dp_count, dp_job, dp_score, dp_sink, j_string, j_first, job_score, job_sink, best_key);
            NVB_LAUNCH_CHECK();
        }
        NVB_TRY(stage(6));
        if (cap) {
            pipe_finalize_dp_kernel<<<jgrid, 256, 0, s>>>(g, dp_count, dp_job, dp_score, dp_sink, dp.t_off, j_string, j_first, best_key,
                                                          best_score, best_pos, rb_strand);
            NVB_LAUNCH_CHECK();
        }
        return launched();
    }

    int extend_per_hit() const
    {
        const uint32_t cap = hit_capacity, hgrid = (cap + 255) / 256;
        if (cap) {
            pipe_expand_hits_kernel<<<(nq + 255) / 256, 256, 0, s>>>(f, g, ranges, sizes, excl, str_len, counts,
                                                                     hit_string, hits.p_off, hits.p_len, hits.t_off, hits.t_len);
            NVB_LAUNCH_CHECK();
        }
        NVB_TRY(stage(4));
        if (dedup && cap) {
            pipe_find_leaders_kernel<<<hgrid, 256, 0, s>>>(counts, hit_string, hits.t_off, hits.t_len, leader, flag);
            NVB_LAUNCH_CHECK();
            size_t bytes = scan_bytes;
            NVB_CUDA_TRY(cub::DeviceScan::ExclusiveSum(scan_tmp, bytes, flag, job_idx, (int)cap, s));
            pipe_job_count_kernel<<<1, 32, 0, s>>>(job_idx, flag, counts);
            NVB_LAUNCH_CHECK();
            pipe_compact_jobs_kernel<<<hgrid, 256, 0, s>>>(counts, flag, job_idx, hits.p_off, hits.p_len, hits.t_off, hits.t_len,
                                                           jobs.p_off, jobs.p_len, jobs.t_off, jobs.t_len);
            NVB_LAUNCH_CHECK();
        }
        NVB_TRY(stage(5));
        NVB_CUDA_TRY(cudaMemsetAsync(best_key, 0, sizeof(unsigned long long) * g.n_reads, s));
        if (cap && dedup) {
            NVB_TRY(score_jobs(jobs, counts + 2, job_score, job_sink));
            pipe_scatter_scores_kernel<<<hgrid, 256, 0, s>>>(g, counts, leader, job_idx, job_score, job_sink, hit_string, h_score, h_sink, best_key);
            NVB_LAUNCH_CHECK();
        } else if (cap)
            NVB_TRY(score_jobs(hits, counts, h_score, h_sink));
        NVB_TRY(stage(6));
        if (cap && !dedup) {
            pipe_reduce_kernel<<<hgrid, 256, 0, s>>>(g, counts, hit_string, h_score, h_sink, best_key);
            NVB_LAUNCH_CHECK();
        }
        pipe_finalize_kernel<<<(g.n_reads + 255) / 256, 256, 0, s>>>(g, best_key, hits.t_off, h_sink, hit_string, best_score, best_pos, rb_strand);
        return launched();
    }

    int best_traceback() const
    {
        const uint32_t rgrid = (g.n_reads + 255) / 256;
        if (per_read || uni) {
            pipe_empty_jobs_kernel<<<rgrid, 256, 0, s>>>(g.n_reads, best.p_off, best.p_len, best.t_off, best.t_len, BA->d_strand);
            NVB_LAUNCH_CHECK();
            const uint32_t jgrid = resident_grid(hit_capacity);
            if (jgrid) {
                pipe_winner_kernel<<<jgrid, 256, 0, s>>>(g, scored(), best_key, best, nullptr, BA->d_strand);
                NVB_LAUNCH_CHECK();
            }
        } else {
            pipe_best_jobs_kernel<<<rgrid, 256, 0, s>>>(g, best_key, hit_string, hits.p_off, hits.p_len, hits.t_off, hits.t_len,
                                                        best.p_off, best.p_len, best.t_off, best.t_len, BA->d_strand);
            NVB_LAUNCH_CHECK();
        }
        if (PP) {
            const uint32_t n_pairs = g.n_reads / 2u;
            pair_empty_rescued_jobs_kernel<<<(n_pairs + 255) / 256, 256, 0, s>>>(n_pairs, PO->d_pair_flags, best.p_len, best.t_len);
            NVB_LAUNCH_CHECK();
        }
        return trace_jobs(best, nullptr, g.n_reads, *BA, 0, best_key);
    }

    int trace_jobs(const Jobs& j, const uint32_t* d_n, uint32_t n, const nvb_best_alignment_out& A, size_t off, const unsigned long long* key) const
    {
        const JobViews v = job_views(j, rd.length + g.band);
        size_t bytes = tb_bytes;
        NVB_TRY(banded_traceback(g.band, P->type, &P->scheme, &v.pats, str_quals, &v.txts, d_n, n, b_score, (nvb_uint2*)b_sink,
                                 (nvb_uint2*)b_source, A.d_ops + off * A.max_ops, A.max_ops, A.d_n_ops + off, tb_tmp, &bytes, s));
        traceback_begin_kernel<<<(n + 255) / 256, 256, 0, s>>>(d_n, n, key, j.t_off, b_source, A.d_n_ops + off, (uint2*)A.d_begin + off);
        return launched();
    }

    Scored scored() const
    {
        if (uni) return *uni;
        return per_read ? Scored{counts + 2, j_string, j_first, jobs, job_score, job_sink} : Scored{counts, hit_string, nullptr, hits, h_score, h_sink};
    }

    int second_best() const
    {
        NVB_CUDA_TRY(cudaMemsetAsync(second_key, 0, sizeof(unsigned long long) * g.n_reads, s));
        if (hit_capacity) {
            const uint32_t grid = resident_grid(hit_capacity);
            pipe_second_reduce_kernel<<<grid, 256, 0, s>>>(g, scored(), str_len, best_pos, rb_strand, MP->d_min_score, second_key);
            NVB_LAUNCH_CHECK();
            if (MO->d_second_pos || MO->d_second_strand) {
                pipe_winner_kernel<<<grid, 256, 0, s>>>(g, scored(), second_key, Jobs{}, MO->d_second_pos, MO->d_second_strand);
                NVB_LAUNCH_CHECK();
            }
        }
        pipe_mapq_kernel<<<(g.n_reads + 255) / 256, 256, 0, s>>>(g, *MP, str_len, best_score, second_key, MO->d_second_score, MO->d_second_pos,
                                                                MO->d_second_strand, MO->d_mapq);
        return launched();
    }

    int cand_segments(bool by_best) const
    {
        const uint32_t cap = hit_capacity, n_reads = g.n_reads;
        NVB_CUDA_TRY(cudaMemsetAsync(cs_cnt, 0, sizeof(uint32_t) * ((size_t)n_reads + 1), s));
        if (cap) {
            const uint32_t grid = resident_grid(cap);
            cand_scatter_kernel<<<grid, 256, 0, s>>>(g, scored(), str_len, MP->d_min_score, nullptr, cs_cnt, nullptr, nullptr, by_best);
            NVB_LAUNCH_CHECK();
            size_t bytes = cs_scan_bytes;
            NVB_CUDA_TRY(cub::DeviceScan::ExclusiveSum(cs_scan_tmp, bytes, cs_cnt, cs_seg, (int)n_reads + 1, s));
            NVB_CUDA_TRY(cudaMemsetAsync(cs_cnt, 0, sizeof(uint32_t) * n_reads, s));
            cand_scatter_kernel<<<grid, 256, 0, s>>>(g, scored(), str_len, MP->d_min_score, cs_seg, cs_cnt, cs_key[0], cs_val[0], by_best);
            NVB_LAUNCH_CHECK();
            bytes = cs_sort_bytes;
            NVB_CUDA_TRY(cub::DeviceSegmentedSort::SortPairs(cs_sort_tmp, bytes, cs_key[0], cs_key[1], cs_val[0], cs_val[1], (int)cap, (int)n_reads,
                                                             cs_seg, cs_seg + 1, s));
        } else
            NVB_CUDA_TRY(cudaMemsetAsync(cs_seg, 0, sizeof(uint32_t) * ((size_t)n_reads + 1), s));
        return NVB_OK;
    }

    int pair_candidates() const
    {
        NVB_CUDA_TRY(cudaMemcpyAsync(se_pos, best_pos, sizeof(uint32_t) * g.n_reads, cudaMemcpyDeviceToDevice, s));
        NVB_TRY(cand_segments(false));
        pair_cand_merge_kernel<<<(g.n_reads + 255) / 256, 256, 0, s>>>(g.n_reads, cs_seg, cs_cnt, cs_key[1], cs_val[1], scored(), pc_end, pc_score,
                                                                        pc_tie, pc_fw, pc_n);
        return launched();
    }

    int all_alignments() const
    {
        const uint32_t n_reads = g.n_reads, acap = AP->capacity, rgrid = (n_reads + 255) / 256;
        const nvb_all_out& O = *AO;
        NVB_TRY(cand_segments(true));
        all_select_kernel<<<rgrid, 256, 0, s>>>(g, scored(), str_len, cs_seg, cs_key[1], cs_val[1], AP->max_per_read, cs_cnt);
        NVB_LAUNCH_CHECK();
        size_t bytes = cs_scan_bytes;
        NVB_CUDA_TRY(cub::DeviceScan::ExclusiveSum(cs_scan_tmp, bytes, cs_cnt, O.d_first, (int)n_reads + 1, s));
        all_count_kernel<<<(n_slices + 256) / 256, 256, 0, s>>>(n_reads, O.d_first, acap, n_slices, O.d_count, al_slice_n);
        NVB_LAUNCH_CHECK();
        if (!acap) return launched();
        all_emit_kernel<<<rgrid, 256, 0, s>>>(g, scored(), O.d_first, cs_seg, cs_val[1], acap, O.d_read, O.d_score, O.d_pos, O.alignment.d_strand,
                                              al_jobs);
        NVB_LAUNCH_CHECK();
        for (uint32_t t = 0; t < n_slices; ++t) {
            const size_t b = (size_t)t * n_reads;
            const Jobs j{al_jobs.p_off + b, al_jobs.p_len + b, al_jobs.t_off + b, al_jobs.t_len + b};
            NVB_TRY(trace_jobs(j, al_slice_n + t, (uint32_t)(acap - b < n_reads ? acap - b : n_reads), O.alignment, b, nullptr));
        }
        return launched();
    }

    int pair_second() const
    {
        const uint32_t n_pairs = g.n_reads / 2u;
        pair_second_kernel<<<(n_pairs + 255) / 256, 256, 0, s>>>(n_pairs, *PP, *MP, str_len, cs_seg, pc_fw, pc_n, pc_end, pc_score, pc_tie,
                                                                  se_pos, rb_strand, best_key, pw_want, pw_idx, pw_toff, rs_score, rs_sink,
                                                                  PO->d_pair_score, PO->d_pair_flags, PO->d_mate_pos, PO->d_mate_strand,
                                                                  PMO->d_second_pair_score, PMO->d_second_mate_pos, PMO->d_second_mate_strand,
                                                                  PMO->d_mate_mapq);
        return launched();
    }

    int paired_rescue() const
    {
        const uint32_t n_reads = g.n_reads, n_pairs = n_reads / 2u, cap = PP->rescue_capacity;
        const uint32_t pgrid = (n_pairs + 255) / 256, sgrid = (n_reads + 255) / 256;
        pair_classify_kernel<<<pgrid, 256, 0, s>>>(g, n_pairs, *PP, best_score, best_pos, rb_strand, str_len, pw_want, pw_pstr, pw_toff, pw_tlen,
                                                    PO->d_pair_score, PO->d_pair_flags, PO->d_mate_score, PO->d_mate_pos, PO->d_mate_strand);
        NVB_LAUNCH_CHECK();
        size_t bytes = pscan_bytes;
        NVB_CUDA_TRY(cub::DeviceScan::ExclusiveSum(pscan_tmp, bytes, pw_want, pw_idx, (int)n_reads, s));
        pipe_count_kernel<<<1, 32, 0, s>>>(pw_idx, pw_want, n_reads, cap, pcounts);
        NVB_LAUNCH_CHECK();
        if (cap) {
            pair_compact_kernel<<<sgrid, 256, 0, s>>>(g, n_reads, cap, pw_want, pw_idx, pw_pstr, pw_toff, pw_tlen, str_len,
                                                      rescue.p_off, rescue.p_len, rescue.t_off, rescue.t_len);
            NVB_LAUNCH_CHECK();
            const JobViews v = job_views(rescue, PP->max_frag);
            size_t fb = full_bytes;
            NVB_TRY(nvb_gotoh_score_indirect(P->type, &P->scheme, &v.pats, str_quals, &v.txts, pcounts, cap, rs_score, (nvb_uint2*)rs_sink, full_tmp, &fb, s));
        }
        pair_finalize_kernel<<<pgrid, 256, 0, s>>>(n_pairs, *PP, pw_want, pw_idx, pw_toff, rs_score, rs_sink, PO->d_pair_score, PO->d_pair_flags,
                                                    PO->d_mate_score, PO->d_mate_pos, PO->d_mate_strand);
        NVB_LAUNCH_CHECK();
        if (PO->d_n_rescue) NVB_CUDA_TRY(cudaMemcpyAsync(PO->d_n_rescue, pcounts, 2 * sizeof(uint32_t), cudaMemcpyDeviceToDevice, s));
        return NVB_OK;
    }

    int after_extension(const uint32_t* hit_counts) const
    {
        if (BA && !PP) NVB_TRY(best_traceback());
        if (MO) NVB_TRY(second_best());
        if (AO) NVB_TRY(all_alignments());
        if (PMO) NVB_TRY(pair_candidates());
        if (PP) NVB_TRY(paired_rescue());
        if (BA && PP) { NVB_TRY(best_traceback()); NVB_TRY(rescue_traceback()); }
        if (PMO) NVB_TRY(pair_second());
        if (n_hits) NVB_CUDA_TRY(cudaMemcpyAsync(n_hits, hit_counts, 3 * sizeof(uint32_t), cudaMemcpyDeviceToDevice, s));
        NVB_TRY(stage(7));
        SE->valid = true;
        return NVB_OK;
    }

    int rescue_traceback() const
    {
        const uint32_t n_pairs = g.n_reads / 2u;
        NVB_CUDA_TRY(cudaMemsetAsync(rt_count, 0, sizeof(uint32_t), s));
        pair_rescue_items_kernel<<<(n_pairs + 255) / 256, 256, 0, s>>>(n_pairs, PO->d_pair_flags, pw_idx, PO->d_mate_strand, rt_items, rt_count,
                                                                       BA->d_strand);
        NVB_LAUNCH_CHECK();
        const JobViews v = job_views(rescue, PP->max_frag);
        FullTbArgs a;
        a.S = make_scheme(&P->scheme); a.pat = make_strset(&v.pats); a.txt = make_strset(&v.txts); a.quals = str_quals;
        a.score = rs_score; a.sink = rs_sink; a.items = rt_items; a.n_items = rt_count;
        a.o.ops = BA->d_ops; a.o.n_ops = BA->d_n_ops; a.o.source = (uint2*)BA->d_begin; a.o.max_ops = BA->max_ops; a.o.absolute = 1u;
        a.pool = rt_pool;
        size_t bytes = rt_pool_bytes;
        return full_warp_traceback(P->type, rd.length, PP->max_frag, &a, &bytes, s);
    }
};

struct ReseedCall {
    const nvb_reseed_params* RP; const nvb_reseed_out* RO;
    uint32_t *map[2], *totals; uint8_t* flag; unsigned long long* key;
    uint32_t *r_words, *r_len; uint8_t* r_quals;
    uint32_t *u_string, *u_tie; Jobs u; int32_t* u_score; uint2* u_sink;
    char* sel_tmp; size_t sel_bytes;

    int carve(const PipeCall& c, void* base, size_t& need)
    {
        const uint32_t n = c.g.n_reads, cap = c.hit_capacity;
        TempCarver tc(base);
        map[0] = tc.take<uint32_t>(n); map[1] = tc.take<uint32_t>(n); flag = tc.take<uint8_t>((size_t)n + 16);
        totals = tc.take<uint32_t>(8); key = tc.take<unsigned long long>(n);
        r_words = tc.take<uint32_t>((size_t)c.g.n_strings * (c.g.stride / (32u / c.g.bits)) + 4); r_len = tc.take<uint32_t>(c.g.n_strings);
        r_quals = c.P->d_read_quals ? tc.take<uint8_t>((size_t)c.g.n_strings * c.g.stride + 16) : nullptr;
        u_string = tc.take<uint32_t>(cap); u_tie = tc.take<uint32_t>(cap); u = take_jobs(tc, cap);
        u_score = tc.take<int32_t>(cap); u_sink = tc.take<uint2>(cap);
        sel_bytes = 0;
        NVB_CUDA_TRY(cub::DeviceSelect::Flagged(nullptr, sel_bytes, map[0], flag, map[1], totals + 4, (int)n, c.s));
        sel_tmp = tc.take<char>(sel_bytes);
        need = tc.total();
        return NVB_OK;
    }

    int run(PipeCall& c)
    {
        const cudaStream_t s = c.s;
        const PipeGeom g0 = c.g;
        const uint32_t n = g0.n_reads, cap = c.hit_capacity, n_rounds = RP->max_reseed + 1u;
        uint32_t* const words0 = c.str_words; uint32_t* const len0 = c.str_len; uint8_t* const quals0 = c.str_quals;
        int32_t* const h_score0 = c.h_score; uint2* const h_sink0 = c.h_sink;
        uint8_t* const rounds = RO ? RO->d_rounds : nullptr; uint32_t* const active = RO ? RO->d_active : nullptr;
        const uint32_t rgrid = (n + 255) / 256;
        NVB_CUDA_TRY(cudaMemsetAsync(totals, 0, 8 * sizeof(uint32_t), s));
        NVB_CUDA_TRY(cudaMemsetAsync(key, 0, sizeof(unsigned long long) * n, s));
        if (rounds) NVB_CUDA_TRY(cudaMemsetAsync(rounds, 1, n, s));
        if (active) NVB_CUDA_TRY(cudaMemsetAsync(active, 0, sizeof(uint32_t) * n_rounds, s));
        reseed_iota_kernel<<<rgrid, 256, 0, s>>>(n, map[0]);
        NVB_LAUNCH_CHECK();
        NVB_TRY(default_stage_events(&c.SE));
        NVB_TRY(c.stage(0));
        NVB_TRY(c.make_strings()); NVB_TRY(c.stage(1));
        uint32_t n_r = n, host[5] = {0u, 0u, 0u, 0u, 0u};
        int cur = 0;
        for (uint32_t r = 0; r < n_rounds && n_r; ++r) {
            const uint32_t kept = host[0], base = host[3];
            c.g.n_reads = n_r; c.g.n_strings = n_r * g0.strands; c.nq = c.g.n_strings * g0.seeds_per_string;
            c.g.seed_offset = reseed_offset(r, g0.seed_interval, RP->max_reseed);
            if (r) {
                reseed_gather_kernel<<<(uint32_t)(((uint64_t)c.g.n_strings * (g0.stride / (32u / g0.bits)) + 255) / 256), 256, 0, s>>>(
                    c.g, map[cur], words0, len0, quals0, r_words, r_len, quals0 ? r_quals : nullptr, rounds, r);
                NVB_LAUNCH_CHECK();
                c.str_words = r_words; c.str_len = r_len; c.str_quals = quals0 ? r_quals : nullptr;
            }
            c.hit_capacity = cap - kept;
            c.h_score = c.hit_score ? c.hit_score + kept : h_score0;
            c.h_sink = c.hit_sink ? (uint2*)c.hit_sink + kept : h_sink0;
            NVB_TRY(c.match_seeds()); NVB_TRY(c.stage(2));
            NVB_TRY(c.hit_slots());   NVB_TRY(c.stage(3));
            NVB_TRY(c.per_read ? c.extend_per_read() : c.extend_per_hit());
            if (c.hit_capacity) {
                if (c.hit_read || c.hit_window) {
                    reseed_export_hits_kernel<<<(c.hit_capacity + 255) / 256, 256, 0, s>>>(c.g, c.counts, map[cur], c.hit_string, c.hits.t_off,
                        c.hits.t_len, c.hit_read ? c.hit_read + kept : nullptr, c.hit_window ? (uint2*)c.hit_window + kept : nullptr);
                    NVB_LAUNCH_CHECK();
                }
                reseed_fold_kernel<<<resident_grid(c.hit_capacity), 256, 0, s>>>(c.g, c.scored(), map[cur], base, kept, u_string, u_tie, u,
                                                                                  u_score, u_sink, key);
                NVB_LAUNCH_CHECK();
            }
            reseed_counts_kernel<<<1, 32, 0, s>>>(c.counts, c.dedup, c.per_read, totals, active, r, n_r);
            NVB_LAUNCH_CHECK();
            if (r + 1u == n_rounds) break;
            reseed_flag_kernel<<<(n_r + 255) / 256, 256, 0, s>>>(c.g, c.ranges, map[cur], c.str_len, key, c.PP ? nullptr : RP->d_min_score,
                                                                 RP->rep_seeds, flag);
            NVB_LAUNCH_CHECK();
            size_t bytes = sel_bytes;
            NVB_CUDA_TRY(cub::DeviceSelect::Flagged(sel_tmp, bytes, map[cur], flag, map[cur ^ 1], totals + 4, (int)n_r, s));
            NVB_CUDA_TRY(cudaMemcpyAsync(host, totals, sizeof(host), cudaMemcpyDeviceToHost, s));
            NVB_CUDA_TRY(cudaStreamSynchronize(s));
            n_r = host[4]; cur ^= 1;
        }
        c.g = g0; c.str_words = words0; c.str_len = len0; c.str_quals = quals0; c.hit_capacity = cap;
        const Scored U{totals + 3, u_string, u_tie, u, u_score, u_sink};
        c.uni = &U; c.best_key = key;
        reseed_best_kernel<<<rgrid, 256, 0, s>>>(n, key, c.best_score, c.best_pos, c.rb_strand);
        NVB_LAUNCH_CHECK();
        if (cap) {
            pipe_winner_kernel<<<resident_grid(cap), 256, 0, s>>>(g0, U, key, Jobs{}, c.best_pos, c.rb_strand);
            NVB_LAUNCH_CHECK();
        }
        return c.after_extension(totals);
    }
};

static int seed_extend_impl(const SeedExtendReq& R, void* d_temp, size_t* temp_bytes, void* stream, ReseedCall* RS = nullptr)
{
    if (!R.reads || !temp_bytes) return NVB_E_INVALID;
    if (R.BA && (!R.BA->d_ops || !R.BA->d_n_ops || !R.BA->d_begin || R.BA->max_ops == 0)) return NVB_E_INVALID;
    if ((R.MP == nullptr) != (R.MO == nullptr && R.PMO == nullptr)) return NVB_E_INVALID;
    if (R.MP && (!R.MP->d_min_score || R.MP->max_read_len < R.reads->length)) return NVB_E_INVALID;
    if (R.MO && (!R.MO->d_second_score || !R.MO->d_mapq)) return NVB_E_INVALID;
    if (R.PMO && (!R.PMO->d_second_pair_score || !R.PMO->d_mate_mapq)) return NVB_E_INVALID;
    if (R.PP && R.BA && R.reads->length > FULL_TB_MAX_M) return NVB_E_UNSUPPORTED;
    if (R.AO && R.reads->length > FULL_TB_MAX_M) return NVB_E_UNSUPPORTED;
    const nvb_seed_extend_params* P = R.P;
    if (R.PP) {
        if (!R.PO->d_pair_score || !R.PO->d_pair_flags || !R.PO->d_mate_score || !R.PO->d_mate_pos || !R.PO->d_mate_strand) return NVB_E_INVALID;
        if (!P || !P->both_strands || (R.n_reads & 1u) || R.PP->max_frag == 0 || R.PP->min_frag > R.PP->max_frag) return NVB_E_INVALID;
    }
    if (!valid_fmindex(R.fmi) || !R.fmi->d_ssa || !R.genome || !valid_strset(R.reads) || !P) return NVB_E_INVALID;
    if (R.reads->bits == 8) return NVB_E_UNSUPPORTED;
    if (P->seed_len == 0 || P->seed_interval == 0 || P->max_seed_hits == 0) return NVB_E_INVALID;
    if (R.n_reads && (!R.best_score || !R.best_pos)) return NVB_E_INVALID;
    const uint32_t max_len = R.reads->length;
    if (max_len < P->seed_len) return NVB_E_INVALID;

    PipeCall c{R};
    PipeGeom& g = c.g;
    g.n_reads = R.n_reads; g.strands = P->both_strands ? 2u : 1u; g.n_strings = R.n_reads * g.strands;
    g.bits = R.reads->bits;
    const uint32_t spw = 32u / g.bits;
    g.stride = (max_len + spw - 1u) / spw * spw;
    g.seeds_per_string = (max_len - P->seed_len) / P->seed_interval + 1u;
    g.seed_len = P->seed_len; g.seed_interval = P->seed_interval; g.band = P->band_len;
    g.max_seed_hits = P->max_seed_hits; g.genome_len = R.fmi->length;
    if ((uint64_t)g.n_strings * g.stride > 0xFFFFFFFFull) return NVB_E_UNSUPPORTED;
    const uint64_t nq64 = (uint64_t)g.n_strings * g.seeds_per_string;
    if (nq64 > 0x7FFFFFFFull) return NVB_E_UNSUPPORTED;
    if (nq64 * (uint64_t)P->max_seed_hits > 0xFFFFFFFFull) return NVB_E_UNSUPPORTED;

    const cudaStream_t s = c.s = as_stream(stream);
    c.f = make_fmindex(R.fmi); c.rd = make_strset(R.reads); c.nq = (uint32_t)nq64;
    if (R.PMO) {
        c.se_mo.d_second_score = R.PMO->d_mate_second_score; c.se_mo.d_mapq = R.PMO->d_mate_mapq;
        c.MO = &c.se_mo;
    }
    c.dedup = P->dedup_jobs != 0;
    c.per_read = c.dedup && g_pipe_path != 1 && !R.hit_read && !R.hit_window && !R.hit_score && !R.hit_sink;
    const nvb_gotoh_scheme& SC = P->scheme;
    c.eligible = c.per_read && P->type == NVB_LOCAL && g.bits == 2 && P->band_len <= 32 && !SC.d_qual_table && SC.match > 0 && SC.mismatch < 0 &&
                 SC.pattern_gap_open < 0 && SC.pattern_gap_ext <= 0 && SC.text_gap_open < 0 && SC.text_gap_ext <= 0;
    c.seed_split = c.per_read && c.f.sa_shift == 0u && c.f.ktab_k && g.seed_len > c.f.ktab_k && g_seed_split;
    size_t need = 0, rs_need = 0;
    NVB_TRY(c.carve(d_temp, need));
    if (RS) NVB_TRY(RS->carve(c, d_temp ? (char*)d_temp + need : nullptr, rs_need));
    need += rs_need;
    if (!d_temp || *temp_bytes < need) { *temp_bytes = need; return NVB_E_TEMP_SIZE; }
    if (R.n_reads == 0) {
        if (RS && RS->RO && RS->RO->d_active) NVB_CUDA_TRY(cudaMemsetAsync(RS->RO->d_active, 0, sizeof(uint32_t) * (RS->RP->max_reseed + 1u), s));
        if (R.AO) {
            NVB_CUDA_TRY(cudaMemsetAsync(R.AO->d_first, 0, sizeof(uint32_t), s));
            NVB_CUDA_TRY(cudaMemsetAsync(R.AO->d_count, 0, 2 * sizeof(uint32_t), s));
        }
        return NVB_OK;
    }

    if (RS) return RS->run(c);
    NVB_TRY(default_stage_events(&c.SE));
    NVB_TRY(c.stage(0));
    NVB_TRY(c.make_strings()); NVB_TRY(c.stage(1));
    NVB_TRY(c.match_seeds());  NVB_TRY(c.stage(2));
    NVB_TRY(c.hit_slots());    NVB_TRY(c.stage(3));
    NVB_TRY(c.per_read ? c.extend_per_read() : c.extend_per_hit());
    if (R.hit_capacity && (R.hit_read || R.hit_window)) {
        pipe_export_hits_kernel<<<(R.hit_capacity + 255) / 256, 256, 0, s>>>(g, c.counts, c.hit_string, c.hits.t_off, c.hits.t_len, R.hit_read,
                                                                             (uint2*)R.hit_window);
        NVB_LAUNCH_CHECK();
    }
    if (!c.dedup) NVB_CUDA_TRY(cudaMemcpyAsync(c.counts + 2, c.counts, sizeof(uint32_t), cudaMemcpyDeviceToDevice, s));
    return c.after_extension(c.counts);
}

extern "C" void nvb_debug_pipeline_path(int path) { g_pipe_path = path; }
extern "C" void nvb_debug_seed_split(int on) { g_seed_split = on; }
extern "C" void nvb_debug_perfect_shortcut(int on) { g_perfect_shortcut = on; }
extern "C" int nvb_debug_dp_jobs(uint32_t* n)
{
    if (!n || !g_last_dp_count) return NVB_E_INVALID;
    NVB_CUDA_TRY(cudaDeviceSynchronize());
    NVB_CUDA_TRY(cudaMemcpy(n, g_last_dp_count, sizeof(uint32_t), cudaMemcpyDeviceToHost));
    return NVB_OK;
}
extern "C" int nvb_debug_seed_todo(uint32_t* n)
{
    if (!n || !g_last_seed_todo) return NVB_E_INVALID;
    uint32_t c[SEED_TODO_LISTS * SEED_TODO_PITCH];
    NVB_CUDA_TRY(cudaDeviceSynchronize());
    NVB_CUDA_TRY(cudaMemcpy(c, g_last_seed_todo, sizeof(c), cudaMemcpyDeviceToHost));
    *n = 0u;
    for (uint32_t l = 0; l < SEED_TODO_LISTS; ++l) *n += c[l * SEED_TODO_PITCH];
    return NVB_OK;
}

extern "C" int nvb_seed_extend(const nvb_fm_index* fmi, const uint32_t* d_genome,
                    const nvb_string_set* reads, uint32_t n_reads,
                    const nvb_seed_extend_params* P, uint32_t hit_capacity,
                    int32_t* d_best_score, uint32_t* d_best_pos,
                    uint32_t* d_n_hits, uint32_t* d_hit_read, nvb_uint2* d_hit_window,
                    int32_t* d_hit_score, nvb_uint2* d_hit_sink,
                    void* d_temp, size_t* temp_bytes, void* stream)
{
    SeedExtendReq R = {};
    R.fmi = fmi; R.genome = d_genome; R.reads = reads; R.n_reads = n_reads; R.P = P; R.hit_capacity = hit_capacity;
    R.best_score = d_best_score; R.best_pos = d_best_pos; R.n_hits = d_n_hits; R.hit_read = d_hit_read; R.hit_window = d_hit_window;
    R.hit_score = d_hit_score; R.hit_sink = d_hit_sink;
    return seed_extend_impl(R, d_temp, temp_bytes, stream);
}

extern "C" int nvb_seed_extend_traceback(const nvb_fm_index* fmi, const uint32_t* d_genome,
                    const nvb_string_set* reads, uint32_t n_reads,
                    const nvb_seed_extend_params* P, uint32_t hit_capacity,
                    int32_t* d_best_score, uint32_t* d_best_pos,
                    uint32_t* d_n_hits, uint32_t* d_hit_read, nvb_uint2* d_hit_window,
                    int32_t* d_hit_score, nvb_uint2* d_hit_sink,
                    const nvb_best_alignment_out* best_alignment,
                    void* d_temp, size_t* temp_bytes, void* stream)
{
    if (!best_alignment) return NVB_E_INVALID;
    SeedExtendReq R = {};
    R.fmi = fmi; R.genome = d_genome; R.reads = reads; R.n_reads = n_reads; R.P = P; R.hit_capacity = hit_capacity;
    R.best_score = d_best_score; R.best_pos = d_best_pos; R.n_hits = d_n_hits; R.hit_read = d_hit_read; R.hit_window = d_hit_window;
    R.hit_score = d_hit_score; R.hit_sink = d_hit_sink; R.BA = best_alignment;
    return seed_extend_impl(R, d_temp, temp_bytes, stream);
}

extern "C" int nvb_seed_extend_paired(const nvb_fm_index* fmi, const uint32_t* d_genome,
                    const nvb_string_set* reads, uint32_t n_pairs,
                    const nvb_seed_extend_params* P, uint32_t hit_capacity,
                    const nvb_pair_params* pair_params, const nvb_pair_out* out,
                    uint32_t* d_n_hits, void* d_temp, size_t* temp_bytes, void* stream)
{
    if (!pair_params || !out || n_pairs > 0x3FFFFFFFu) return NVB_E_INVALID;
    SeedExtendReq R = {};
    R.fmi = fmi; R.genome = d_genome; R.reads = reads; R.n_reads = 2u * n_pairs; R.P = P; R.hit_capacity = hit_capacity;
    R.best_score = out->d_mate_score; R.best_pos = out->d_mate_pos; R.n_hits = d_n_hits; R.PP = pair_params; R.PO = out;
    return seed_extend_impl(R, d_temp, temp_bytes, stream);
}

extern "C" int nvb_seed_extend_mapq(const nvb_fm_index* fmi, const uint32_t* d_genome,
                    const nvb_string_set* reads, uint32_t n_reads,
                    const nvb_seed_extend_params* P, uint32_t hit_capacity,
                    int32_t* d_best_score, uint32_t* d_best_pos,
                    uint32_t* d_n_hits, uint32_t* d_hit_read, nvb_uint2* d_hit_window,
                    int32_t* d_hit_score, nvb_uint2* d_hit_sink,
                    const nvb_best_alignment_out* best_alignment,
                    const nvb_mapq_params* mapq, const nvb_mapq_out* mapq_out,
                    void* d_temp, size_t* temp_bytes, void* stream)
{
    if (!mapq || !mapq_out) return NVB_E_INVALID;
    SeedExtendReq R = {};
    R.fmi = fmi; R.genome = d_genome; R.reads = reads; R.n_reads = n_reads; R.P = P; R.hit_capacity = hit_capacity;
    R.best_score = d_best_score; R.best_pos = d_best_pos; R.n_hits = d_n_hits; R.hit_read = d_hit_read; R.hit_window = d_hit_window;
    R.hit_score = d_hit_score; R.hit_sink = d_hit_sink; R.BA = best_alignment; R.MP = mapq; R.MO = mapq_out;
    return seed_extend_impl(R, d_temp, temp_bytes, stream);
}

extern "C" int nvb_seed_extend_reseed(const nvb_fm_index* fmi, const uint32_t* d_genome,
                    const nvb_string_set* reads, uint32_t n_reads,
                    const nvb_seed_extend_params* P, uint32_t hit_capacity,
                    int32_t* d_best_score, uint32_t* d_best_pos,
                    uint32_t* d_n_hits, uint32_t* d_hit_read, nvb_uint2* d_hit_window,
                    int32_t* d_hit_score, nvb_uint2* d_hit_sink,
                    const nvb_best_alignment_out* best_alignment,
                    const nvb_mapq_params* mapq, const nvb_mapq_out* mapq_out,
                    const nvb_reseed_params* reseed, const nvb_reseed_out* reseed_out,
                    void* d_temp, size_t* temp_bytes, void* stream)
{
    if (!reseed || !reseed->d_min_score || !reads || reseed->max_read_len < reads->length) return NVB_E_INVALID;
    if (reseed->max_reseed > 254u) return NVB_E_INVALID;
    if (P && reseed->max_reseed && P->seed_interval < reseed->max_reseed + 1u) return NVB_E_INVALID;
    SeedExtendReq R = {};
    R.fmi = fmi; R.genome = d_genome; R.reads = reads; R.n_reads = n_reads; R.P = P; R.hit_capacity = hit_capacity;
    R.best_score = d_best_score; R.best_pos = d_best_pos; R.n_hits = d_n_hits; R.hit_read = d_hit_read; R.hit_window = d_hit_window;
    R.hit_score = d_hit_score; R.hit_sink = d_hit_sink; R.BA = best_alignment; R.MP = mapq; R.MO = mapq_out;
    ReseedCall RS = {};
    RS.RP = reseed; RS.RO = reseed_out;
    return seed_extend_impl(R, d_temp, temp_bytes, stream, &RS);
}

extern "C" int nvb_seed_extend_all(const nvb_fm_index* fmi, const uint32_t* d_genome,
                    const nvb_string_set* reads, uint32_t n_reads,
                    const nvb_seed_extend_params* P, uint32_t hit_capacity,
                    int32_t* d_best_score, uint32_t* d_best_pos,
                    uint32_t* d_n_hits, uint32_t* d_hit_read, nvb_uint2* d_hit_window,
                    int32_t* d_hit_score, nvb_uint2* d_hit_sink,
                    const nvb_best_alignment_out* best_alignment,
                    const nvb_mapq_params* mapq, const nvb_mapq_out* mapq_out,
                    const nvb_all_params* all_params, const nvb_all_out* all_out,
                    void* d_temp, size_t* temp_bytes, void* stream)
{
    if (!mapq || !mapq_out || !all_params || !all_out || best_alignment) return NVB_E_INVALID;
    const nvb_all_out& O = *all_out;
    const nvb_best_alignment_out& A = O.alignment;
    if (!O.d_first || !O.d_read || !O.d_score || !O.d_pos || !O.d_count || !A.d_ops || !A.d_n_ops || !A.d_begin || !A.d_strand || A.max_ops == 0)
        return NVB_E_INVALID;
    SeedExtendReq R = {};
    R.fmi = fmi; R.genome = d_genome; R.reads = reads; R.n_reads = n_reads; R.P = P; R.hit_capacity = hit_capacity;
    R.best_score = d_best_score; R.best_pos = d_best_pos; R.n_hits = d_n_hits; R.hit_read = d_hit_read; R.hit_window = d_hit_window;
    R.hit_score = d_hit_score; R.hit_sink = d_hit_sink; R.MP = mapq; R.MO = mapq_out; R.AP = all_params; R.AO = all_out;
    return seed_extend_impl(R, d_temp, temp_bytes, stream);
}

extern "C" int nvb_seed_extend_paired_mapq(const nvb_fm_index* fmi, const uint32_t* d_genome,
                    const nvb_string_set* reads, uint32_t n_pairs,
                    const nvb_seed_extend_params* P, uint32_t hit_capacity,
                    const nvb_pair_params* pair_params, const nvb_pair_out* out,
                    const nvb_mapq_params* mapq, const nvb_pair_mapq_out* mapq_out,
                    uint32_t* d_n_hits, void* d_temp, size_t* temp_bytes, void* stream)
{
    if (!pair_params || !out || !mapq || !mapq_out || n_pairs > 0x3FFFFFFFu) return NVB_E_INVALID;
    SeedExtendReq R = {};
    R.fmi = fmi; R.genome = d_genome; R.reads = reads; R.n_reads = 2u * n_pairs; R.P = P; R.hit_capacity = hit_capacity;
    R.best_score = out->d_mate_score; R.best_pos = out->d_mate_pos; R.n_hits = d_n_hits; R.PP = pair_params; R.PO = out; R.MP = mapq; R.PMO = mapq_out;
    return seed_extend_impl(R, d_temp, temp_bytes, stream);
}

extern "C" int nvb_seed_extend_paired_traceback(const nvb_fm_index* fmi, const uint32_t* d_genome,
                    const nvb_string_set* reads, uint32_t n_pairs,
                    const nvb_seed_extend_params* P, uint32_t hit_capacity,
                    const nvb_pair_params* pair_params, const nvb_pair_out* out,
                    const nvb_best_alignment_out* mate_alignment,
                    const nvb_mapq_params* mapq, const nvb_pair_mapq_out* mapq_out,
                    uint32_t* d_n_hits, void* d_temp, size_t* temp_bytes, void* stream)
{
    if (!pair_params || !out || !mate_alignment || n_pairs > 0x3FFFFFFFu) return NVB_E_INVALID;
    SeedExtendReq R = {};
    R.fmi = fmi; R.genome = d_genome; R.reads = reads; R.n_reads = 2u * n_pairs; R.P = P; R.hit_capacity = hit_capacity;
    R.best_score = out->d_mate_score; R.best_pos = out->d_mate_pos; R.n_hits = d_n_hits; R.PP = pair_params; R.PO = out;
    R.BA = mate_alignment; R.MP = mapq; R.PMO = mapq_out;
    return seed_extend_impl(R, d_temp, temp_bytes, stream);
}

extern "C" int nvb_seed_extend_paired_reseed(const nvb_fm_index* fmi, const uint32_t* d_genome,
                    const nvb_string_set* reads, uint32_t n_pairs,
                    const nvb_seed_extend_params* P, uint32_t hit_capacity,
                    const nvb_pair_params* pair_params, const nvb_pair_out* out,
                    const nvb_best_alignment_out* mate_alignment,
                    const nvb_mapq_params* mapq, const nvb_pair_mapq_out* mapq_out,
                    const nvb_reseed_params* reseed, const nvb_reseed_out* reseed_out,
                    uint32_t* d_n_hits, void* d_temp, size_t* temp_bytes, void* stream)
{
    if (!pair_params || !out || n_pairs > 0x3FFFFFFFu) return NVB_E_INVALID;
    if (!reseed || reseed->max_reseed > 254u) return NVB_E_INVALID;
    if (P && reseed->max_reseed && P->seed_interval < reseed->max_reseed + 1u) return NVB_E_INVALID;
    SeedExtendReq R = {};
    R.fmi = fmi; R.genome = d_genome; R.reads = reads; R.n_reads = 2u * n_pairs; R.P = P; R.hit_capacity = hit_capacity;
    R.best_score = out->d_mate_score; R.best_pos = out->d_mate_pos; R.n_hits = d_n_hits; R.PP = pair_params; R.PO = out;
    R.BA = mate_alignment; R.MP = mapq; R.PMO = mapq_out;
    ReseedCall RS = {};
    RS.RP = reseed; RS.RO = reseed_out;
    return seed_extend_impl(R, d_temp, temp_bytes, stream, &RS);
}

extern "C" int nvb_debug_mapq_eval(const int32_t* d_best, const uint8_t* d_has_second, const int32_t* d_second, const uint32_t* d_len,
                                   const int32_t* d_match_bonus, const int32_t* d_min_score, uint32_t n, uint8_t* d_mapq, void* stream)
{
    if (!n) return NVB_OK;
    if (!d_best || !d_has_second || !d_second || !d_len || !d_match_bonus || !d_min_score || !d_mapq) return NVB_E_INVALID;
    debug_mapq_eval_kernel<<<(n + 255) / 256, 256, 0, as_stream(stream)>>>(d_best, d_has_second, d_second, d_len, d_match_bonus, d_min_score, n, d_mapq);
    return launched();
}
```

nvbio_b200/csrc/pipeline_core.cuh:

```cuda
#pragma once
#include "fm_core.cuh"

namespace nvb {

__host__ __device__ __forceinline__ uint32_t nvb_clz(uint32_t x) {
#ifdef __CUDA_ARCH__
    return (uint32_t)__clz((int)x);
#else
    return (uint32_t)__builtin_clz(x);
#endif
}

__host__ __device__ __forceinline__ uint32_t job_diff_bits(const uint32_t* __restrict__ str_words, const uint32_t* __restrict__ genome,
                                                           const uint32_t po, const uint32_t t, const uint32_t i, const uint32_t cnt)
{
    const uint32_t x = (be2_window(str_words, po + i, cnt) ^ be2_window(genome, t + i, cnt)) >> (32u - 2u * cnt);
    return (x | (x >> 1)) & 0x55555555u;
}
__host__ __device__ __forceinline__ uint32_t job_differences(const uint32_t* __restrict__ str_words, const uint32_t* __restrict__ genome,
                                                             const uint32_t po, const uint32_t M, const uint32_t t, const uint32_t limit)
{
    uint32_t mm = 0;
    for (uint32_t i = 0; i < M && mm <= limit; i += 16u) mm += nvb_popc(job_diff_bits(str_words, genome, po, t, i, M - i < 16u ? M - i : 16u));
    return mm;
}

__host__ __device__ __forceinline__ uint32_t diff_row_mask(const uint32_t w0, const uint32_t cnt, const uint32_t lo, const uint32_t hi)
{
    const uint32_t a = lo > w0 ? lo : w0, b = hi < w0 + cnt - 1u ? hi : w0 + cnt - 1u;
    if (a > b) return 0u;
    return ((2u << (2u * (w0 + cnt - 1u - a))) - 1u) & ~((1u << (2u * (w0 + cnt - 1u - b))) - 1u);
}
__host__ __device__ inline void job_diff_span(const uint32_t* __restrict__ str_words, const uint32_t* __restrict__ genome, const uint32_t po,
                                              const uint32_t t, const uint32_t lo, const uint32_t hi, int32_t& first, int32_t& last)
{
    first = (int32_t)hi + 1; last = (int32_t)lo - 1;
    for (uint32_t i = lo; i <= hi; i += 16u) {
        const uint32_t cnt = hi + 1u - i < 16u ? hi + 1u - i : 16u;
        const uint32_t d = job_diff_bits(str_words, genome, po, t, i, cnt);
        if (!d) continue;
        if (first > (int32_t)hi) first = (int32_t)(i + cnt - 1u - ((31u - nvb_clz(d)) >> 1));
        last = (int32_t)(i + cnt - 1u - ((31u - nvb_clz(d & (0u - d))) >> 1));
    }
}
__host__ __device__ __forceinline__ uint32_t text_window16(const uint32_t g0, const uint32_t g1, const uint32_t g2, const uint32_t g3, const uint32_t off)
{
    const uint32_t idx = off >> 4, sh = 2u * (off & 15u);
    const uint32_t hi = idx == 0u ? g0 : (idx == 1u ? g1 : g2), lo = idx == 0u ? g1 : (idx == 1u ? g2 : g3);
    return sh ? ((hi << sh) | (lo >> (32u - sh))) : hi;
}

constexpr uint32_t SHORTCUT_WORDS = 10;

__host__ __device__ inline bool gapless_job_shortcut(const uint32_t* __restrict__ str_words, const uint32_t* __restrict__ genome,
                                                     const uint32_t po, const uint32_t M, const uint32_t to, const uint32_t N, const uint32_t band,
                                                     const int32_t match, const int32_t mismatch, const int32_t max_gap_open,
                                                     int32_t& score, uint32_t& sink_x, uint32_t& sink_y, const bool one_gap = true)
{
    if (M < 1u || to == 0u || N < M + band - 1u) return false;
    const uint32_t j0 = band / 2u;
    const int32_t o = -max_gap_open, lim = !one_gap ? o : (o + match - mismatch < 2 * o ? o + match - mismatch : 2 * o);
    const uint32_t mm_max = (uint32_t)((lim - 1) / match);
    int32_t h = 0, best = 0, f1 = (int32_t)M, f2 = (int32_t)M, l1 = -1, l2 = -1; uint32_t end = 0, prev = 0, mm0 = 0;
    const uint32_t wr = po >> 4, wt = (to + j0) >> 4, sht = 2u * ((to + j0) & 15u), wlast = (to + N - 1u) >> 4;
    for (uint32_t kb = 0; kb * 16u < M && mm0 <= mm_max; kb += SHORTCUT_WORDS) {
        uint32_t rw[SHORTCUT_WORDS], tw[SHORTCUT_WORDS + 1];
#pragma unroll
        for (uint32_t q = 0; q < SHORTCUT_WORDS; ++q) rw[q] = (kb + q) * 16u < M ? str_words[wr + kb + q] : 0u;
#pragma unroll
        for (uint32_t q = 0; q <= SHORTCUT_WORDS; ++q) tw[q] = wt + kb + q <= wlast ? genome[wt + kb + q] : 0u;
#pragma unroll
        for (uint32_t q = 0; q < SHORTCUT_WORDS; ++q) {
            const uint32_t i = (kb + q) * 16u;
            if (i >= M || mm0 > mm_max) break;
            const uint32_t cnt = M - i < 16u ? M - i : 16u;
            const uint32_t x = (rw[q] ^ (sht ? (tw[q] << sht) | (tw[q + 1] >> (32u - sht)) : tw[q])) >> (32u - 2u * cnt);
            uint32_t d = (x | (x >> 1)) & 0x55555555u;
            while (d && mm0 <= mm_max) {
                const uint32_t bit = 31u - nvb_clz(d);
                const uint32_t p = i + (cnt - 1u - (bit >> 1));
                d &= ~(1u << bit);
                h += match * (int32_t)(p - prev);
                if (h >= best) { best = h; end = p; }
                h += mismatch; h = h > 0 ? h : 0;
                if (mm0 == 0u) f1 = (int32_t)p; else if (mm0 == 1u) f2 = (int32_t)p;
                l2 = l1; l1 = (int32_t)p;
                prev = p + 1u; ++mm0;
            }
        }
    }
    if (mm0 > mm_max) return false;
    h += match * (int32_t)(M - prev);
    if (h >= best) { best = h; end = M; }
    const int32_t delta = match * (int32_t)M - best;
    if (delta >= lim) return false;
    const bool gap1 = delta >= o;
    const uint32_t U = gap1 ? (uint32_t)((delta - o) / match) : 0u;
    if (gap1 && 2u * U + 1u > M) return false;
    const uint32_t hi = M - 1u - U;
    int32_t fa = f1 >= (int32_t)U ? f1 : (f2 >= (int32_t)U ? f2 : (int32_t)(M - U)), ba = l1 <= (int32_t)hi ? l1 : (l2 <= (int32_t)hi ? l2 : (int32_t)U - 1);
    fa = fa > (int32_t)hi ? (int32_t)(M - U) : fa; ba = ba < (int32_t)U ? (int32_t)U - 1 : ba;
    int32_t fb = INT_MIN, bb = INT_MAX; uint32_t fd = j0, bd = j0;
    const bool perfect = (mm0 == 0u);
    const uint32_t t = (uint32_t)(delta / match);
    const uint32_t c16 = M < 16u ? M : 16u;
    const uint32_t r0 = be2_window(str_words, po, c16) >> (32u - 2u * c16);
    const uint32_t wi = to >> 4, r = to & 15u, wl = (to + N - 1u) >> 4;
    const uint32_t g0 = genome[wi], g1 = (wi + 1u <= wl) ? genome[wi + 1u] : 0u;
    const uint32_t g2 = (wi + 2u <= wl) ? genome[wi + 2u] : 0u, g3 = (wi + 3u <= wl) ? genome[wi + 3u] : 0u;
    uint32_t rE = 0, e0 = 0, e1 = 0, e2 = 0, e3 = 0, mF = 0, mB = 0;
    const uint32_t te = to + M - c16, we = te >> 4;
    if (gap1) {
        rE = be2_window(str_words, po + M - c16, c16) >> (32u - 2u * c16);
        e0 = genome[we]; e1 = (we + 1u <= wl) ? genome[we + 1u] : 0u; e2 = (we + 2u <= wl) ? genome[we + 2u] : 0u; e3 = (we + 3u <= wl) ? genome[we + 3u] : 0u;
        mF = diff_row_mask(0u, c16, U, hi); mB = diff_row_mask(M - c16, c16, U, hi);
    }
    uint32_t jtop = j0;
    for (uint32_t jj = 0; jj < band; ++jj) {
        if (jj == j0) continue;
        const uint32_t x = (text_window16(g0, g1, g2, g3, r + jj) >> (32u - 2u * c16)) ^ r0, dx = (x | (x >> 1)) & 0x55555555u;
        if (gap1) {
            const uint32_t y = (text_window16(e0, e1, e2, e3, (te & 15u) + jj) >> (32u - 2u * c16)) ^ rE, dy = (y | (y >> 1)) & 0x55555555u & mB;
            int32_t F, B;
            if ((dx & mF) && dy) { F = (int32_t)(c16 - 1u - ((31u - nvb_clz(dx & mF)) >> 1)); B = (int32_t)(M - 1u - ((31u - nvb_clz(dy & (0u - dy))) >> 1)); }
            else job_diff_span(str_words, genome, po, to + jj, U, hi, F, B);
            if (F > fa) { fb = fa; fa = F; fd = jj; } else if (F > fb) fb = F;
            if (B < ba) { bb = ba; ba = B; bd = jj; } else if (B < bb) bb = B;
        }
        if (nvb_popc(dx) > t) continue;
        if (job_differences(str_words, genome, po, M, to + jj, t) > t) continue;
        if (!perfect) return false;
        if (jj > jtop) jtop = jj;
    }
    if (gap1 && (fd != bd ? (int64_t)ba - fa : ((int64_t)ba - fb < (int64_t)bb - fa ? (int64_t)ba - fb : (int64_t)bb - fa)) <= (int64_t)U - 1) return false;
    score = best;
    if (perfect) { sink_x = M + jtop; sink_y = M; }
    else         { sink_x = end + j0; sink_y = end; }
    return true;
}

__host__ __device__ __forceinline__ bool distinct_alignment(uint32_t p, uint32_t t, uint32_t bp, uint32_t bt, uint32_t len)
{
    const uint32_t d = len / 2u;
    return t != bt || p < bp - (bp < d ? bp : d) || p > bp + d;
}

__host__ __device__ __forceinline__ unsigned long long make_best_key(int32_t score, uint32_t index)
{
    return ((unsigned long long)((uint32_t)score ^ 0x80000000u) << 32) | (unsigned long long)(0xFFFFFFFFu - index);
}
__host__ __device__ __forceinline__ int32_t  best_key_score(unsigned long long key) { return (int32_t)((uint32_t)(key >> 32) ^ 0x80000000u); }
__host__ __device__ __forceinline__ uint32_t best_key_index(unsigned long long key) { return 0xFFFFFFFFu - (uint32_t)(key & 0xFFFFFFFFull); }

__host__ __device__ __forceinline__ bool job_aligned(uint2 sink) { return sink.x != 0xFFFFFFFFu; }

__host__ __device__ __forceinline__ bool reportable(int32_t score, uint2 sink, int32_t min_score) { return job_aligned(sink) && score >= min_score; }

__host__ __device__ __forceinline__ uint32_t reseed_offset(uint32_t round, uint32_t seed_interval, uint32_t max_reseed)
{
    return round * (seed_interval / (max_reseed + 1u));
}

__host__ __device__ __forceinline__ bool reseed_read(uint32_t range_sum, uint32_t range_count, uint32_t rep_seeds, bool aligned)
{
    return range_count == 0u || range_sum >= rep_seeds * range_count || !aligned;
}

__host__ __device__ __forceinline__ unsigned long long end_strand(uint32_t end, uint32_t strand) { return ((unsigned long long)end << 1) | (strand & 1u); }

__host__ __device__ inline uint32_t select_distinct(unsigned long long* es, uint32_t* idx, uint32_t n, uint32_t len, uint32_t k)
{
    uint32_t m = 0;
    for (uint32_t i = 0; i < n && (k == 0u || m < k); ++i) {
        const unsigned long long c = es[i];
        const uint32_t p = (uint32_t)(c >> 1), t = (uint32_t)(c & 1u);
        bool ok = true;
        for (uint32_t a = 0; a < m && ok; ++a) ok = distinct_alignment(p, t, (uint32_t)(es[a] >> 1), (uint32_t)(es[a] & 1u), len);
        if (!ok) continue;
        const uint32_t j = idx[i];
        es[m] = c; idx[m] = j; ++m;
    }
    return m;
}

__host__ __device__ __forceinline__ uint32_t aln_begin(uint32_t end, uint32_t len) { return end > len ? end - len : 0u; }

__host__ __device__ __forceinline__ bool fr_concordant(uint32_t fb, uint32_t fe, uint32_t rb, uint32_t re, uint32_t min_frag, uint32_t max_frag)
{
    return fb <= rb && fe <= re && re > fb && (re - fb) >= min_frag && (re - fb) <= max_frag;
}

struct PairSecond {
    uint32_t star_end[2], star_strand[2], len[2];
    bool has; int32_t score; uint32_t end[2], strand[2], tie[2];

    __host__ __device__ __forceinline__ void init(uint32_t e1, uint32_t t1, uint32_t l1, uint32_t e2, uint32_t t2, uint32_t l2)
    {
        star_end[0] = e1; star_strand[0] = t1; len[0] = l1; star_end[1] = e2; star_strand[1] = t2; len[1] = l2;
        has = false; score = INT_MIN; end[0] = end[1] = 0xFFFFFFFFu; strand[0] = strand[1] = 0u; tie[0] = tie[1] = 0xFFFFFFFFu;
    }
    __host__ __device__ __forceinline__ void offer(int32_t s, uint32_t e1, uint32_t t1, uint32_t i1, uint32_t e2, uint32_t t2, uint32_t i2)
    {
        if (!distinct_alignment(e1, t1, star_end[0], star_strand[0], len[0]) && !distinct_alignment(e2, t2, star_end[1], star_strand[1], len[1]))
            return;
        if (has && (s < score || (s == score && (i1 > tie[0] || (i1 == tie[0] && i2 >= tie[1]))))) return;
        has = true; score = s; end[0] = e1; strand[0] = t1; tie[0] = i1; end[1] = e2; strand[1] = t2; tie[1] = i2;
    }
    __host__ __device__ __forceinline__ void offer_rescue(int a, int32_t s, uint32_t ae, uint32_t at, uint32_t ai, uint32_t oe)
    {
        if (a == 0) offer(s, ae, at, ai, oe, 1u - at, 0xFFFFFFFFu);
        else        offer(s, oe, 1u - at, 0xFFFFFFFFu, ae, at, ai);
    }
};

struct MateCands { const uint32_t* end; const int32_t* score; const uint32_t* tie; uint32_t n_fw, n, len; };

__host__ __device__ __forceinline__ uint32_t lower_bound_end(const uint32_t* end, uint32_t lo, uint32_t hi, uint64_t v)
{
    while (lo < hi) { const uint32_t mid = (lo + hi) >> 1; if ((uint64_t)end[mid] < v) lo = mid + 1; else hi = mid; }
    return lo;
}

__host__ __device__ inline void pair_combinations(const MateCands m[2], uint32_t min_frag, uint32_t max_frag, PairSecond& ps)
{
    for (int a = 0; a < 2; ++a) {
        const MateCands& F = m[a]; const MateCands& R = m[1 - a];
        for (uint32_t i = 0; i < F.n_fw; ++i) {
            const uint32_t fe = F.end[i], fb = aln_begin(fe, F.len);
            uint32_t k = lower_bound_end(R.end, R.n_fw, R.n, (uint64_t)fb + min_frag);
            for (; k < R.n && (uint64_t)R.end[k] <= (uint64_t)fb + max_frag; ++k) {
                const uint32_t re = R.end[k];
                if (!fr_concordant(fb, fe, aln_begin(re, R.len), re, min_frag, max_frag)) continue;
                const int32_t s = F.score[i] + R.score[k];
                if (a == 0) ps.offer(s, fe, 0u, F.tie[i], re, 1u, R.tie[k]);
                else        ps.offer(s, re, 1u, R.tie[k], fe, 0u, F.tie[i]);
            }
        }
    }
}

__host__ __device__ inline uint32_t bowtie_mapq2(int32_t best_score, bool has_second, int32_t second_score, int32_t perfect, int32_t min_score,
                                                 bool monotone)
{
    const float max_s = (float)perfect, min_s = (float)min_score;
    const float diff = max_s - min_s;
    const float best = (float)best_score;
    if (best < min_s) return 0;
    const float best_over = best - min_s;
    const bool top = best_over == diff;
    if (monotone) {
        if (!has_second) {
            if      (best_over >= diff * 0.8f) return 42;
            else if (best_over >= diff * 0.7f) return 40;
            else if (best_over >= diff * 0.6f) return 24;
            else if (best_over >= diff * 0.5f) return 23;
            else if (best_over >= diff * 0.4f) return 8;
            else if (best_over >= diff * 0.3f) return 3;
            return 0;
        }
        const float best_diff = fabsf(fabsf(best) - fabsf((float)second_score));
        if      (best_diff >= diff * 0.9f) return top ? 39 : 33;
        else if (best_diff >= diff * 0.8f) return top ? 38 : 27;
        else if (best_diff >= diff * 0.7f) return top ? 37 : 26;
        else if (best_diff >= diff * 0.6f) return top ? 36 : 22;
        else if (best_diff >= diff * 0.5f) return top ? 35 : best_over >= diff * 0.84f ? 25 : best_over >= diff * 0.68f ? 16 : 5;
        else if (best_diff >= diff * 0.4f) return top ? 34 : best_over >= diff * 0.84f ? 21 : best_over >= diff * 0.68f ? 14 : 4;
        else if (best_diff >= diff * 0.3f) return top ? 32 : best_over >= diff * 0.88f ? 18 : best_over >= diff * 0.67f ? 15 : 3;
        else if (best_diff >= diff * 0.2f) return top ? 31 : best_over >= diff * 0.88f ? 17 : best_over >= diff * 0.67f ? 11 : 0;
        else if (best_diff >= diff * 0.1f) return top ? 30 : best_over >= diff * 0.88f ? 12 : best_over >= diff * 0.67f ? 7 : 0;
        else if (best_diff > 0.0f)         return best_over >= diff * 0.67f ? 6 : 2;
        return best_over >= diff * 0.67f ? 1 : 0;
    }
    if (!has_second) {
        if      (best_over >= diff * 0.8f) return 44;
        else if (best_over >= diff * 0.7f) return 42;
        else if (best_over >= diff * 0.6f) return 41;
        else if (best_over >= diff * 0.5f) return 36;
        else if (best_over >= diff * 0.4f) return 28;
        else if (best_over >= diff * 0.3f) return 24;
        return 22;
    }
    const float best_diff = fabsf(fabsf(best) - fabsf((float)second_score));
    if      (best_diff >= diff * 0.9f) return 40;
    else if (best_diff >= diff * 0.8f) return 39;
    else if (best_diff >= diff * 0.7f) return 38;
    else if (best_diff >= diff * 0.6f) return 37;
    else if (best_diff >= diff * 0.5f) return top ? 35 : best_over >= diff * 0.5f ? 25 : 20;
    else if (best_diff >= diff * 0.4f) return top ? 34 : best_over >= diff * 0.5f ? 21 : 19;
    else if (best_diff >= diff * 0.3f) return top ? 33 : best_over >= diff * 0.5f ? 18 : 16;
    else if (best_diff >= diff * 0.2f) return top ? 32 : best_over >= diff * 0.5f ? 17 : 12;
    else if (best_diff >= diff * 0.1f) return top ? 31 : best_over >= diff * 0.5f ? 14 : 9;
    else if (best_diff > 0.0f)         return best_over >= diff * 0.5f ? 11 : 2;
    return best_over >= diff * 0.5f ? 1 : 0;
}

__host__ __device__ inline uint32_t full_traceback_first_row(int type, uint32_t sink_x, uint32_t sink_y, int32_t score, int32_t s_max,
                                                             int32_t go, int32_t ge)
{
    if (type != NVB_LOCAL || go >= 0 || ge >= 0) return 0u;
    const int64_t g = go > ge ? go : ge;
    const int64_t room = (int64_t)sink_y * (s_max > 0 ? s_max : 0) - (int64_t)score;
    const int64_t span = (int64_t)sink_y + (room > 0 ? room / -g : 0);
    return span < (int64_t)sink_x ? (uint32_t)((int64_t)sink_x - span) : 0u;
}

}
```

Before: 448.6.

## Compact seed ranges into 32-bit records with side table for true SA ranges

Seed match results are stored as 32-bit records: unique located hits encode the genome position directly, empty ranges use a sentinel, and multi-hit ranges go to a warp-compacted side array allocated through an atomic counter. The resolve and reseed kernels read these records with wider vector loads, which halves the per-seed traffic. The deferred todo list now carries the partial range (q,x,y) so the wide kernel no longer rereads ranges. The 2-bit read packing kernel also writes forward and reverse-complement words in one thread per read. The cost is extra atomics and ballots in the seed kernels and an indirect load for multi-hit ranges.

After: 468.7 (median of 6 runs). 4.5% higher.

```diff
diff --git a/include/nvbio_b200_debug.h b/include/nvbio_b200_debug.h
--- a/include/nvbio_b200_debug.h
+++ b/include/nvbio_b200_debug.h
@@ -19,6 +19,8 @@
 
 void nvb_debug_seed_split(int on);
 int nvb_debug_seed_todo(uint32_t* n);
+void nvb_debug_seed_records(int on);
+int nvb_debug_seed_layout(int* records);
 
 void nvb_debug_perfect_shortcut(int on);
 int nvb_debug_dp_jobs(uint32_t* n);
diff --git a/nvbio_b200/_lib.py b/nvbio_b200/_lib.py
--- a/nvbio_b200/_lib.py
+++ b/nvbio_b200/_lib.py
@@ -19,7 +19,7 @@
     "nvb_debug_gotoh_last_route", "nvb_debug_force_gotoh_path", "nvb_debug_full_minb", "nvb_debug_full_warp", "nvb_debug_full_traceback_warp",
     "nvb_debug_pair_format", "nvb_debug_pair_rows2", "nvb_debug_traceback_fast", "nvb_debug_pair_extra_smem",
     "nvb_debug_pipeline_path", "nvb_debug_seed_split", "nvb_debug_seed_todo", "nvb_debug_perfect_shortcut", "nvb_debug_dp_jobs", "nvb_debug_mapq_eval",
-    "nvb_debug_bgzf_grid",
+    "nvb_debug_bgzf_grid", "nvb_debug_seed_records", "nvb_debug_seed_layout",
 ]
 
 
diff --git a/nvbio_b200/csrc/pipeline.cu b/nvbio_b200/csrc/pipeline.cu
--- a/nvbio_b200/csrc/pipeline.cu
+++ b/nvbio_b200/csrc/pipeline.cu
@@ -78,35 +78,59 @@
 pipe_make_strings_2bit_be_kernel(const StrSet reads, const PipeGeom g, uint32_t* __restrict__ out_words, uint32_t* __restrict__ out_len)
 {
     const uint32_t words_per_string = g.stride / 16u;
-    const uint64_t t = (uint64_t)blockIdx.x * 256 + threadIdx.x, total = (uint64_t)g.n_strings * words_per_string;
+    const uint64_t t = (uint64_t)blockIdx.x * 256 + threadIdx.x, total = (uint64_t)g.n_reads * words_per_string;
     if (t >= total) return;
-    uint32_t s, w;
-    if (total <= 0xFFFFFFFFull) { s = (uint32_t)t / words_per_string; w = (uint32_t)t - s * words_per_string; }
-    else                        { s = (uint32_t)(t / words_per_string); w = (uint32_t)(t % words_per_string); }
-    const uint32_t read = s / g.strands, strand = s % g.strands;
-    const uint32_t off = str_off(reads, read), len = str_len(reads, read);
-    if (w == 0) out_len[s] = len;
+    uint32_t read, w;
+    if (total <= 0xFFFFFFFFull) { read = (uint32_t)t / words_per_string; w = (uint32_t)t - read * words_per_string; }
+    else                        { read = (uint32_t)(t / words_per_string); w = (uint32_t)(t % words_per_string); }
+    const bool both = g.strands > 1u;
+    const uint32_t s = read * g.strands, off = str_off(reads, read), len = str_len(reads, read);
+    if (w == 0) { out_len[s] = len; if (both) out_len[s + 1u] = len; }
     const uint32_t first = w * 16u;
-    uint32_t word = 0;
+    uint32_t fw = 0, rc = 0;
     if (first < len) {
         const uint32_t cnt = (len - first) < 16u ? (len - first) : 16u;
-        if (strand == 0) {
-            word = load16_2bit_be(reads.words, off + first, cnt);
-        } else {
+        fw = load16_2bit_be(reads.words, off + first, cnt);
+        if (both) {
             const uint32_t lo = len - first - cnt;
-            uint32_t x = load16_2bit_be(reads.words, off + lo, cnt);
-            x = revcomp16_2bit(x);
-            word = x << (2u * (16u - cnt));
-        }
-        if (cnt < 16u) word &= ~(0xFFFFFFFFu >> (2u * cnt));
-    }
-    out_words[t] = word;
+            const uint32_t x = revcomp16_2bit(load16_2bit_be(reads.words, off + lo, cnt));
+            rc = x << (2u * (16u - cnt));
+        }
+        if (cnt < 16u) { const uint32_t pad = ~(0xFFFFFFFFu >> (2u * cnt)); fw &= pad; rc &= pad; }
+    }
+    out_words[(size_t)s * words_per_string + w] = fw;
+    if (both) out_words[(size_t)(s + 1u) * words_per_string + w] = rc;
 }
 
 __device__ __forceinline__ uint32_t seed_range_hits(uint2 range, uint32_t max_seed_hits)
 {
     const uint32_t sz = (range.y == 0xFFFFFFFFu) ? 1u : ((range.x <= range.y) ? (range.y - range.x + 1u) : 0u);
     return sz < max_seed_hits ? sz : max_seed_hits;
+}
+
+struct Seeds { uint2* ranges; uint32_t* rec; uint2* side; uint32_t* side_n; };
+
+template <bool REC>
+__device__ __forceinline__ uint2 seed_range(const Seeds& o, const size_t q) { return REC ? seed_record_range(o.rec[q], o.side) : o.ranges[q]; }
+
+template <bool REC>
+__device__ __forceinline__ void store_seed(const Seeds& o, const uint32_t q, const uint32_t x, const uint32_t y, const bool live)
+{
+    if (!REC) {
+        if (live) o.ranges[q] = make_uint2(x, y);
+        return;
+    }
+    const bool side = live && seed_record_needs_side(x, y);
+    const uint32_t m = __ballot_sync(0xFFFFFFFFu, side);
+    uint32_t i = 0;
+    if (m) {
+        const uint32_t lane = threadIdx.x & 31u, first = (uint32_t)__ffs(m) - 1u;
+        uint32_t base = 0;
+        if (lane == first) base = atomicAdd(o.side_n, (uint32_t)__popc(m));
+        i = __shfl_sync(0xFFFFFFFFu, base, (int)first) + (uint32_t)__popc(m & ((1u << lane) - 1u));
+        if (side) o.side[i] = make_uint2(x, y);
+    }
+    if (live) o.rec[q] = seed_record(x, y, i);
 }
 
 __device__ __forceinline__ uint2 hit_window(uint32_t pos, uint32_t seed_begin, uint32_t len, const PipeGeom& g)
@@ -121,18 +145,17 @@
 constexpr uint32_t SEED_TODO_LISTS = 64;
 constexpr uint32_t SEED_TODO_PITCH = 32;
 constexpr uint32_t SEED_ITER = 8;
-template <int BITS, bool DEFER>
+template <int BITS, bool DEFER, bool REC>
 __global__ void __launch_bounds__(SEED_BLOCK, 2048 / SEED_BLOCK)
 pipe_seed_match_kernel(const FmIndex f, const PipeGeom g, const uint32_t* __restrict__ words, const uint32_t* __restrict__ slen,
-                       const uint32_t* __restrict__ genome, uint2* __restrict__ ranges, uint32_t* __restrict__ sizes,
-                       uint32_t* __restrict__ todo, uint32_t* __restrict__ todo_count)
+                       const uint32_t* __restrict__ genome, const Seeds o, uint32_t* __restrict__ sizes,
+                       uint3* __restrict__ todo, uint32_t* __restrict__ todo_count)
 {
     constexpr uint32_t ITER = DEFER ? SEED_ITER : 1u;
 #pragma unroll 1
     for (uint32_t it = 0; it < ITER; ++it) {
         const uint32_t q = (blockIdx.x * ITER + it) * SEED_BLOCK + threadIdx.x;
         const bool live = q < g.n_strings * g.seeds_per_string;
-        if (!DEFER && !live) return;
         uint32_t x = 1, y = 0;
         bool deferred = false;
         if (live) {
@@ -147,9 +170,9 @@
                 } else
                     fm_match_one<BITS, true>(f, words, s * g.stride + pos, g.seed_len, 0u, x, y);
             }
-            ranges[q] = make_uint2(x, y);
             if (sizes && !deferred) sizes[q] = seed_range_hits(make_uint2(x, y), g.max_seed_hits);
         }
+        store_seed<REC>(o, q, x, y, live && !deferred);
         if (DEFER) {
             const uint32_t m = __ballot_sync(0xFFFFFFFFu, deferred);
             if (m) {
@@ -158,28 +181,31 @@
                 uint32_t base = 0;
                 if (lane == 0) base = atomicAdd(todo_count + list * SEED_TODO_PITCH, (uint32_t)__popc(m));
                 base = __shfl_sync(0xFFFFFFFFu, base, 0);
-                if (deferred) todo[(size_t)list * cap + base + __popc(m & ((1u << lane) - 1u))] = q;
+                if (deferred) todo[(size_t)list * cap + base + __popc(m & ((1u << lane) - 1u))] = make_uint3(q, x, y);
             }
         }
     }
 }
-template <int BITS>
+template <int BITS, bool REC>
 __global__ void __launch_bounds__(SEED_BLOCK, 2048 / SEED_BLOCK)
 pipe_seed_match_wide_kernel(const FmIndex f, const PipeGeom g, const uint32_t* __restrict__ words,
-                            const uint32_t* __restrict__ genome, uint2* __restrict__ ranges, uint32_t* __restrict__ sizes,
-                            const uint32_t* __restrict__ todo, const uint32_t* __restrict__ todo_count, const uint32_t seed_grid)
+                            const uint32_t* __restrict__ genome, const Seeds o, uint32_t* __restrict__ sizes,
+                            const uint3* __restrict__ todo, const uint32_t* __restrict__ todo_count, const uint32_t seed_grid)
 {
     const uint32_t list = blockIdx.x % SEED_TODO_LISTS, per_list = gridDim.x / SEED_TODO_LISTS;
     const uint32_t cap = ((seed_grid + SEED_TODO_LISTS - 1u) / SEED_TODO_LISTS) * SEED_BLOCK * SEED_ITER;
     const uint32_t n = todo_count[list * SEED_TODO_PITCH];
-    for (uint32_t t = (blockIdx.x / SEED_TODO_LISTS) * SEED_BLOCK + threadIdx.x; t < n; t += per_list * SEED_BLOCK) {
-        const uint32_t q = todo[(size_t)list * cap + t];
-        const uint32_t s = q / g.seeds_per_string, k = q % g.seeds_per_string;
-        const uint2 r = ranges[q];
-        uint32_t x = r.x, y = r.y;
-        if (fm_match_locate_one<BITS, true, FM_RESUME>(f, genome, words, s * g.stride + g.seed_offset + k * g.seed_interval, g.seed_len, x, y) == FM_EMPTY) { x = 1; y = 0; }
-        ranges[q] = make_uint2(x, y);
-        if (sizes) sizes[q] = seed_range_hits(make_uint2(x, y), g.max_seed_hits);
+    for (uint32_t t0 = (blockIdx.x / SEED_TODO_LISTS) * SEED_BLOCK + (threadIdx.x & ~31u); t0 < n; t0 += per_list * SEED_BLOCK) {
+        const uint32_t t = t0 + (threadIdx.x & 31u);
+        uint32_t q = 0, x = 1, y = 0;
+        if (t < n) {
+            const uint3 e = todo[(size_t)list * cap + t];
+            q = e.x; x = e.y; y = e.z;
+            const uint32_t s = q / g.seeds_per_string, k = q % g.seeds_per_string;
+            if (fm_match_locate_one<BITS, true, FM_RESUME>(f, genome, words, s * g.stride + g.seed_offset + k * g.seed_interval, g.seed_len, x, y) == FM_EMPTY) { x = 1; y = 0; }
+            if (sizes) sizes[q] = seed_range_hits(make_uint2(x, y), g.max_seed_hits);
+        }
+        store_seed<REC>(o, q, x, y, t < n);
     }
 }
 
@@ -235,10 +261,33 @@
 using RjTileState = cub::ScanTileState<uint32_t>;
 using RjPrefixOp  = cub::TilePrefixCallbackOp<uint32_t, ::cuda::std::plus<uint32_t>, RjTileState>;
 
-template <uint32_t RB>
-__device__ __forceinline__ uint32_t range_batch(const uint2* __restrict__ rr, const uint32_t q0, const uint32_t n, const bool vec,
+template <uint32_t RB, bool REC>
+__device__ __forceinline__ uint32_t range_batch(const Seeds& o, const size_t base, const uint32_t q0, const uint32_t n, const bool vec,
                                                 const uint32_t max_seed_hits, uint32_t& hits)
 {
+    uint32_t m = 0;
+    if (REC) {
+        const uint32_t* rr = o.rec + base;
+        uint32_t v[RB];
+        if (vec) {
+#pragma unroll
+            for (uint32_t j = 0; j < RB; j += 4u) {
+                const uint4 w = q0 + j < n ? *reinterpret_cast<const uint4*>(rr + q0 + j) : make_uint4(SEED_REC_EMPTY, SEED_REC_EMPTY, SEED_REC_EMPTY, SEED_REC_EMPTY);
+                v[j] = w.x; v[j + 1] = w.y; v[j + 2] = w.z; v[j + 3] = w.w;
+            }
+        } else {
+#pragma unroll
+            for (uint32_t j = 0; j < RB; ++j) v[j] = q0 + j < n ? rr[q0 + j] : SEED_REC_EMPTY;
+        }
+#pragma unroll
+        for (uint32_t j = 0; j < RB; ++j) {
+            const uint32_t sz = v[j] < SEED_REC_SIDE ? 1u : (v[j] == SEED_REC_EMPTY ? 0u : seed_range_hits(seed_record_range(v[j], o.side), max_seed_hits));
+            hits += sz;
+            m |= (sz != 0u ? 1u : 0u) << j;
+        }
+        return m;
+    }
+    const uint2* rr = o.ranges + base;
     uint2 v[RB];
     if (vec) {
 #pragma unroll
@@ -250,7 +299,6 @@
 #pragma unroll
         for (uint32_t j = 0; j < RB; ++j) v[j] = q0 + j < n ? rr[q0 + j] : make_uint2(1u, 0u);
     }
-    uint32_t m = 0;
 #pragma unroll
     for (uint32_t j = 0; j < RB; ++j) {
         const uint32_t sz = seed_range_hits(v[j], max_seed_hits);
@@ -267,8 +315,9 @@
     if (blockIdx.x == 0 && threadIdx.x == 0) { counts[2] = 0u; counts[3] = 0u; *dp_count = 0u; }
 }
 
+template <bool REC>
 __global__ void __launch_bounds__(RJ_BLOCK, 8)
-pipe_resolve_reads_kernel(const FmIndex f, const PipeGeom g, const uint2* __restrict__ ranges, const uint32_t* __restrict__ slen,
+pipe_resolve_reads_kernel(const FmIndex f, const PipeGeom g, const Seeds o, const uint32_t* __restrict__ slen,
                           const uint32_t hit_capacity, RjTileState tiles, const uint32_t n_tiles, uint32_t* __restrict__ counts,
                           const int shortcut, const int32_t match, const int32_t mismatch, const int32_t max_gap_open,
                           const uint32_t* __restrict__ str_words, const uint32_t* __restrict__ genome,
@@ -291,13 +340,14 @@
     const uint32_t tile = s_tile, r0 = tile * RJ_BLOCK, r = r0 + threadIdx.x;
     const uint32_t per_read = g.strands * g.seeds_per_string;
     const bool live = r < g.n_reads;
-    const uint2* rr = ranges + (size_t)r * per_read;
-
-    const bool vec = ((per_read | (uint32_t)((size_t)ranges >> 3)) & 1u) == 0u;
+    const size_t rr = (size_t)r * per_read;
+
+    constexpr uint32_t RB = REC ? 32u : 16u, PER16 = REC ? 4u : 2u;
+    const bool vec = ((per_read | (uint32_t)(REC ? (size_t)o.rec >> 2 : (size_t)o.ranges >> 3)) & (PER16 - 1u)) == 0u;
     uint32_t hits = 0, run = 0, nonempty = 0;
     if (live)
-        for (uint32_t q0 = 0; q0 < per_read; q0 += 16u) {
-            const uint32_t m = range_batch<16>(rr, q0, per_read, vec, g.max_seed_hits, hits);
+        for (uint32_t q0 = 0; q0 < per_read; q0 += RB) {
+            const uint32_t m = range_batch<RB, REC>(o, rr, q0, per_read, vec, g.max_seed_hits, hits);
             if (q0 < 32u) nonempty |= m << q0;
         }
     if (tile == 0) {
@@ -321,14 +371,14 @@
         for (uint32_t q0 = 0; q0 < per_read; q0 += 32u) {
             uint32_t m = q0 ? 0u : nonempty, unused = 0;
             if (q0)
-                for (uint32_t b = 0; b < 32u; b += 8u) m |= range_batch<8>(rr, q0 + b, per_read, vec, g.max_seed_hits, unused) << b;
+                for (uint32_t b = 0; b < 32u; b += 8u) m |= range_batch<8, REC>(o, rr, q0 + b, per_read, vec, g.max_seed_hits, unused) << b;
             while (m) {
                 uint32_t bq[RJ_BATCH], nb = 0;
                 uint2 brq[RJ_BATCH];
 #pragma unroll
                 for (uint32_t e = 0; e < RJ_BATCH; ++e) { bq[e] = m ? q0 + (uint32_t)__ffs(m) - 1u : 0u; nb += m ? 1u : 0u; m &= m - 1u; }
 #pragma unroll
-                for (uint32_t e = 0; e < RJ_BATCH; ++e) brq[e] = e < nb ? rr[bq[e]] : make_uint2(1u, 0u);
+                for (uint32_t e = 0; e < RJ_BATCH; ++e) brq[e] = e < nb ? seed_range<REC>(o, rr + bq[e]) : make_uint2(1u, 0u);
                 for (uint32_t e = 0; e < nb; ++e) {
                     const uint32_t q = bq[0];
                     const uint2 rq = brq[0];
@@ -616,18 +666,19 @@
     }
 }
 
-__global__ void __launch_bounds__(256)
-reseed_flag_kernel(const PipeGeom g, const uint2* __restrict__ ranges, const uint32_t* __restrict__ map, const uint32_t* __restrict__ str_len,
+template <bool REC>
+__global__ void __launch_bounds__(256)
+reseed_flag_kernel(const PipeGeom g, const Seeds o, const uint32_t* __restrict__ map, const uint32_t* __restrict__ str_len,
                    const unsigned long long* __restrict__ key, const int32_t* __restrict__ min_score, const uint32_t rep_seeds,
                    uint8_t* __restrict__ flag)
 {
     const uint32_t i = blockIdx.x * 256 + threadIdx.x;
     if (i >= g.n_reads) return;
     const uint32_t per_read = g.strands * g.seeds_per_string;
-    const uint2* rr = ranges + (size_t)i * per_read;
+    const size_t rr = (size_t)i * per_read;
     uint32_t range_sum = 0u, range_count = 0u;
     for (uint32_t q = 0; q < per_read; ++q) {
-        const uint2 v = rr[q];
+        const uint2 v = seed_range<REC>(o, rr + q);
         if (v.y != 0xFFFFFFFFu && v.x > v.y) continue;
         range_sum += v.y == 0xFFFFFFFFu ? 1u : v.y - v.x + 1u;
         ++range_count;
@@ -1058,6 +1109,8 @@
 static const uint32_t* g_last_dp_count = nullptr;
 static int g_seed_split = 1;
 static const uint32_t* g_last_seed_todo = nullptr;
+static int g_seed_records = 1;
+static int g_last_seed_records = -1;
 static int g_pipe_path = 0;
 
 #define NVB_TRY(expr) do { const int _r = (expr); if (_r != NVB_OK) return _r; } while (0)
@@ -1082,10 +1135,11 @@
     uint32_t nq;
     bool dedup, per_read, eligible;
     bool seed_split;
+    bool seed_rec;
     nvb_mapq_out se_mo;
     StageEvents* SE;
     uint32_t *str_words, *str_len; uint8_t* str_quals;
-    uint2* ranges; uint32_t *sizes, *excl, *counts, *seed_todo, *seed_todo_n;
+    Seeds seeds; uint32_t *sizes, *excl, *counts, *seed_todo_n; uint3* seed_todo;
     char* rj_tiles; size_t rj_tile_bytes;
     uint32_t *j_string, *j_first;
     uint32_t *leader, *flag, *job_idx;
@@ -1131,10 +1185,12 @@
         str_words = tc.take<uint32_t>((size_t)g.n_strings * (g.stride / (32u / g.bits)) + 4);
         str_len   = tc.take<uint32_t>(g.n_strings);
         str_quals = P->d_read_quals ? tc.take<uint8_t>((size_t)g.n_strings * g.stride + 16) : nullptr;
-        ranges = tc.take<uint2>(nq);
+        if (seed_rec) { seeds.rec = tc.take<uint32_t>(nq); seeds.side = tc.take<uint2>(nq); }
+        else seeds.ranges = tc.take<uint2>(nq);
         if (!per_read) { sizes = tc.take<uint32_t>(nq); excl = tc.take<uint32_t>(nq); }
-        if (seed_split) seed_todo = tc.take<uint32_t>((size_t)nq + (SEED_TODO_LISTS + 1u) * SEED_BLOCK * SEED_ITER);
-        counts = tc.take<uint32_t>(4); seed_todo_n = tc.take<uint32_t>(SEED_TODO_LISTS * SEED_TODO_PITCH);
+        if (seed_split) seed_todo = tc.take<uint3>((size_t)nq + (SEED_TODO_LISTS + 1u) * SEED_BLOCK * SEED_ITER);
+        counts = tc.take<uint32_t>(4); seed_todo_n = tc.take<uint32_t>((SEED_TODO_LISTS + 1u) * SEED_TODO_PITCH);
+        seeds.side_n = seed_todo_n ? seed_todo_n + SEED_TODO_LISTS * SEED_TODO_PITCH : nullptr;
         if (per_read) {
             NVB_CUDA_TRY(RjTileState::AllocationSize((int)((n_reads + RJ_BLOCK - 1u) / RJ_BLOCK), rj_tile_bytes));
             rj_tiles = tc.take<char>(rj_tile_bytes);
@@ -1210,7 +1266,8 @@
     int make_strings() const
     {
         const uint32_t grid = (uint32_t)(((uint64_t)g.n_strings * (g.stride / (32u / g.bits)) + 255) / 256);
-        if (g.bits == 2 && rd.big_endian) pipe_make_strings_2bit_be_kernel<<<grid, 256, 0, s>>>(rd, g, str_words, str_len);
+        const uint32_t grid_be = (uint32_t)(((uint64_t)g.n_reads * (g.stride / 16u) + 255) / 256);
+        if (g.bits == 2 && rd.big_endian) pipe_make_strings_2bit_be_kernel<<<grid_be, 256, 0, s>>>(rd, g, str_words, str_len);
         else if (g.bits == 2)             pipe_make_strings_kernel<2><<<grid, 256, 0, s>>>(rd, g, str_words, str_len);
         else                              pipe_make_strings_kernel<4><<<grid, 256, 0, s>>>(rd, g, str_words, str_len);
         NVB_LAUNCH_CHECK();
@@ -1220,21 +1277,28 @@
 
     int match_seeds() const
     {
+        g_last_seed_records = seed_rec ? 1 : 0;
+        return seed_rec ? match_seeds_as<true>() : match_seeds_as<false>();
+    }
+    template <bool REC>
+    int match_seeds_as() const
+    {
         const uint32_t grid = (nq + SEED_BLOCK - 1) / SEED_BLOCK;
         const uint32_t* loc_genome = (per_read && f.sa_shift == 0u) ? genome : nullptr;
         if (seed_split) {
-            NVB_CUDA_TRY(cudaMemsetAsync(seed_todo_n, 0, SEED_TODO_LISTS * SEED_TODO_PITCH * sizeof(uint32_t), s));
+            NVB_CUDA_TRY(cudaMemsetAsync(seed_todo_n, 0, (SEED_TODO_LISTS * SEED_TODO_PITCH + (REC ? 1u : 0u)) * sizeof(uint32_t), s));
             const uint32_t grid1 = (grid + SEED_ITER - 1u) / SEED_ITER;
-            if (g.bits == 2) pipe_seed_match_kernel<2, true><<<grid1, SEED_BLOCK, 0, s>>>(f, g, str_words, str_len, loc_genome, ranges, sizes, seed_todo, seed_todo_n);
-            else             pipe_seed_match_kernel<4, true><<<grid1, SEED_BLOCK, 0, s>>>(f, g, str_words, str_len, loc_genome, ranges, sizes, seed_todo, seed_todo_n);
+            if (g.bits == 2) pipe_seed_match_kernel<2, true, REC><<<grid1, SEED_BLOCK, 0, s>>>(f, g, str_words, str_len, loc_genome, seeds, sizes, seed_todo, seed_todo_n);
+            else             pipe_seed_match_kernel<4, true, REC><<<grid1, SEED_BLOCK, 0, s>>>(f, g, str_words, str_len, loc_genome, seeds, sizes, seed_todo, seed_todo_n);
             NVB_LAUNCH_CHECK();
             const uint32_t wgrid = (sm_count() * 16u + SEED_TODO_LISTS - 1u) / SEED_TODO_LISTS * SEED_TODO_LISTS;
-            if (g.bits == 2) pipe_seed_match_wide_kernel<2><<<wgrid, SEED_BLOCK, 0, s>>>(f, g, str_words, loc_genome, ranges, sizes, seed_todo, seed_todo_n, grid1);
-            else             pipe_seed_match_wide_kernel<4><<<wgrid, SEED_BLOCK, 0, s>>>(f, g, str_words, loc_genome, ranges, sizes, seed_todo, seed_todo_n, grid1);
+            if (g.bits == 2) pipe_seed_match_wide_kernel<2, REC><<<wgrid, SEED_BLOCK, 0, s>>>(f, g, str_words, loc_genome, seeds, sizes, seed_todo, seed_todo_n, grid1);
+            else             pipe_seed_match_wide_kernel<4, REC><<<wgrid, SEED_BLOCK, 0, s>>>(f, g, str_words, loc_genome, seeds, sizes, seed_todo, seed_todo_n, grid1);
             g_last_seed_todo = seed_todo_n;
         } else {
-            if (g.bits == 2) pipe_seed_match_kernel<2, false><<<grid, SEED_BLOCK, 0, s>>>(f, g, str_words, str_len, loc_genome, ranges, sizes, nullptr, nullptr);
-            else             pipe_seed_match_kernel<4, false><<<grid, SEED_BLOCK, 0, s>>>(f, g, str_words, str_len, loc_genome, ranges, sizes, nullptr, nullptr);
+            if (REC) NVB_CUDA_TRY(cudaMemsetAsync(seeds.side_n, 0, sizeof(uint32_t), s));
+            if (g.bits == 2) pipe_seed_match_kernel<2, false, REC><<<grid, SEED_BLOCK, 0, s>>>(f, g, str_words, str_len, loc_genome, seeds, sizes, nullptr, nullptr);
+            else             pipe_seed_match_kernel<4, false, REC><<<grid, SEED_BLOCK, 0, s>>>(f, g, str_words, str_len, loc_genome, seeds, sizes, nullptr, nullptr);
         }
         return launched();
     }
@@ -1258,9 +1322,9 @@
         NVB_LAUNCH_CHECK();
         const int shortcut = eligible ? g_perfect_shortcut : 0;
         const int32_t max_gap_open = SC.pattern_gap_open > SC.text_gap_open ? SC.pattern_gap_open : SC.text_gap_open;
-        pipe_resolve_reads_kernel<<<n_tiles, RJ_BLOCK, 0, s>>>(f, g, ranges, str_len, cap, tiles, n_tiles, counts, shortcut, SC.match,
-                SC.mismatch, max_gap_open, str_words, genome, j_string, j_first, jobs, job_score, job_sink, dp, dp_job, dp_count,
-                best_key, best_score, best_pos, rb_strand);
+        (seed_rec ? pipe_resolve_reads_kernel<true> : pipe_resolve_reads_kernel<false>)<<<n_tiles, RJ_BLOCK, 0, s>>>(f, g, seeds, str_len,
+                cap, tiles, n_tiles, counts, shortcut, SC.match, SC.mismatch, max_gap_open, str_words, genome, j_string, j_first, jobs,
+                job_score, job_sink, dp, dp_job, dp_count, best_key, best_score, best_pos, rb_strand);
         NVB_LAUNCH_CHECK();
         g_last_dp_count = dp_count;
         NVB_TRY(stage(4)); NVB_TRY(stage(5));
@@ -1283,7 +1347,7 @@
     {
         const uint32_t cap = hit_capacity, hgrid = (cap + 255) / 256;
         if (cap) {
-            pipe_expand_hits_kernel<<<(nq + 255) / 256, 256, 0, s>>>(f, g, ranges, sizes, excl, str_len, counts,
+            pipe_expand_hits_kernel<<<(nq + 255) / 256, 256, 0, s>>>(f, g, seeds.ranges, sizes, excl, str_len, counts,
                                                                      hit_string, hits.p_off, hits.p_len, hits.t_off, hits.t_len);
             NVB_LAUNCH_CHECK();
         }
@@ -1569,8 +1633,8 @@
             reseed_counts_kernel<<<1, 32, 0, s>>>(c.counts, c.dedup, c.per_read, totals, active, r, n_r);
             NVB_LAUNCH_CHECK();
             if (r + 1u == n_rounds) break;
-            reseed_flag_kernel<<<(n_r + 255) / 256, 256, 0, s>>>(c.g, c.ranges, map[cur], c.str_len, key, c.PP ? nullptr : RP->d_min_score,
-                                                                 RP->rep_seeds, flag);
+            (c.seed_rec ? reseed_flag_kernel<true> : reseed_flag_kernel<false>)<<<(n_r + 255) / 256, 256, 0, s>>>(c.g, c.seeds, map[cur],
+                c.str_len, key, c.PP ? nullptr : RP->d_min_score, RP->rep_seeds, flag);
             NVB_LAUNCH_CHECK();
             size_t bytes = sel_bytes;
             NVB_CUDA_TRY(cub::DeviceSelect::Flagged(sel_tmp, bytes, map[cur], flag, map[cur ^ 1], totals + 4, (int)n_r, s));
@@ -1639,6 +1703,7 @@
     c.eligible = c.per_read && P->type == NVB_LOCAL && g.bits == 2 && P->band_len <= 32 && !SC.d_qual_table && SC.match > 0 && SC.mismatch < 0 &&
                  SC.pattern_gap_open < 0 && SC.pattern_gap_ext <= 0 && SC.text_gap_open < 0 && SC.text_gap_ext <= 0;
     c.seed_split = c.per_read && c.f.sa_shift == 0u && c.f.ktab_k && g.seed_len > c.f.ktab_k && g_seed_split;
+    c.seed_rec = c.per_read && c.f.sa_shift == 0u && seed_records_fit(g.genome_len, nq64) && g_seed_records;
     size_t need = 0, rs_need = 0;
     NVB_TRY(c.carve(d_temp, need));
     if (RS) NVB_TRY(RS->carve(c, d_temp ? (char*)d_temp + need : nullptr, rs_need));
@@ -1671,6 +1736,13 @@
 
 extern "C" void nvb_debug_pipeline_path(int path) { g_pipe_path = path; }
 extern "C" void nvb_debug_seed_split(int on) { g_seed_split = on; }
+extern "C" void nvb_debug_seed_records(int on) { g_seed_records = on; }
+extern "C" int nvb_debug_seed_layout(int* records)
+{
+    if (!records || g_last_seed_records < 0) return NVB_E_INVALID;
+    *records = g_last_seed_records;
+    return NVB_OK;
+}
 extern "C" void nvb_debug_perfect_shortcut(int on) { g_perfect_shortcut = on; }
 extern "C" int nvb_debug_dp_jobs(uint32_t* n)
 {
diff --git a/nvbio_b200/csrc/pipeline_core.cuh b/nvbio_b200/csrc/pipeline_core.cuh
--- a/nvbio_b200/csrc/pipeline_core.cuh
+++ b/nvbio_b200/csrc/pipeline_core.cuh
@@ -156,6 +156,24 @@
 
 __host__ __device__ __forceinline__ bool reportable(int32_t score, uint2 sink, int32_t min_score) { return job_aligned(sink) && score >= min_score; }
 
+constexpr uint32_t SEED_REC_EMPTY = 0xFFFFFFFFu;
+constexpr uint32_t SEED_REC_SIDE  = 0xC0000000u;
+__host__ __device__ __forceinline__ bool seed_records_fit(uint64_t text_len, uint64_t n_seeds)
+{
+    return text_len < SEED_REC_SIDE && n_seeds <= (SEED_REC_EMPTY & ~SEED_REC_SIDE);
+}
+__host__ __device__ __forceinline__ uint32_t seed_record(uint32_t x, uint32_t y, uint32_t side_i)
+{
+    return y == 0xFFFFFFFFu ? x : (x > y ? SEED_REC_EMPTY : (SEED_REC_SIDE | side_i));
+}
+__host__ __device__ __forceinline__ bool seed_record_needs_side(uint32_t x, uint32_t y) { return y != 0xFFFFFFFFu && x <= y; }
+__host__ __device__ __forceinline__ uint2 seed_record_range(uint32_t rec, const uint2* __restrict__ side)
+{
+    if (rec == SEED_REC_EMPTY) return make_uint2(1u, 0u);
+    if (rec < SEED_REC_SIDE) return make_uint2(rec, 0xFFFFFFFFu);
+    return side[rec & ~SEED_REC_SIDE];
+}
+
 __host__ __device__ __forceinline__ uint32_t reseed_offset(uint32_t round, uint32_t seed_interval, uint32_t max_reseed)
 {
     return round * (seed_interval / (max_reseed + 1u));
```
